# cmeraki/audiotoken

Hardware: AMD Instinct MI355X
Metric: audio-sec tokenized / wall-sec (acoustic + semantic_m) (higher is better)
Workload: dtype f32 (linear layers: two fp16 pieces per operand, three MFMA products, fp32 accumulate)

## Files before the change

audiotoken_amd/_cabi.py:

```python
from __future__ import annotations

import ctypes as C
import os
from pathlib import Path

import numpy as np

_LIB_PATH = Path(__file__).resolve().parent / "lib" / "libaudiotoken_hip.so"
_lib = None


class HipLibraryError(RuntimeError):
    pass


class SegmentDesc(C.Structure):
    _fields_ = [("pcm", C.c_void_p), ("table", C.c_void_p), ("chunk_off", C.c_int64), ("chunk_len", C.c_int32), ("out_start", C.c_int32),
                ("valid_len", C.c_int32), ("fmt", C.c_int32), ("scale", C.c_float), ("o", C.c_int32), ("n", C.c_int32), ("width", C.c_int32),
                ("chunk_out_len", C.c_int32)]


PCM_S16, PCM_S32, PCM_F32, PCM_U8 = 0, 1, 2, 3


class ResampleRow(C.Structure):
    _fields_ = [("pcm", C.c_void_p), ("table", C.c_void_p), ("src_base", C.c_int64), ("src_len", C.c_int64), ("src_total", C.c_int64),
                ("out_start", C.c_int64), ("out_len", C.c_int32), ("fmt", C.c_int32), ("scale", C.c_float), ("o", C.c_int32), ("n", C.c_int32),
                ("width", C.c_int32), ("final", C.c_int32), ("reserved", C.c_int32), ("dst_off", C.c_int64)]


class PcmRowDesc(C.Structure):
    _fields_ = [("src_off", C.c_int64), ("dst_off", C.c_int64), ("n", C.c_int64), ("scale", C.c_float), ("reserved", C.c_int32)]


class FlacRowDesc(C.Structure):
    _fields_ = [("src_off", C.c_int64), ("n", C.c_int64), ("first_block", C.c_int32), ("scale", C.c_float)]


class FlacBlock(C.Structure):
    _fields_ = [("first", C.c_int64), ("byte_off", C.c_int64), ("row", C.c_int32), ("n", C.c_int32), ("kind", C.c_int32), ("order", C.c_int32),
                ("porder", C.c_int32), ("nbytes", C.c_int32)]


FLAC_BLOCK = 4096
FLAC_CONSTANT, FLAC_VERBATIM, FLAC_FIXED = 0, 1, 2
FLAC_BLOCK_DTYPE = np.dtype([("first", "<i8"), ("byte_off", "<i8"), ("row", "<i4"), ("n", "<i4"), ("kind", "<i4"), ("order", "<i4"), ("porder", "<i4"),
                             ("nbytes", "<i4")])


class GemmDesc(C.Structure):
    _fields_ = [
        ("X", C.c_void_p), ("x_bstride", C.c_int64), ("Tin", C.c_int32), ("Cin", C.c_int32), ("ldx", C.c_int32),
        ("ktaps", C.c_int32), ("stride", C.c_int32), ("pad_left", C.c_int32), ("pad_mode", C.c_int32),
        ("W", C.c_void_p), ("bias", C.c_void_p),
        ("C", C.c_void_p), ("c_bstride", C.c_int64), ("ldc", C.c_int32),
        ("R", C.c_void_p), ("r_bstride", C.c_int64), ("ldr", C.c_int32),
        ("M", C.c_int32), ("N", C.c_int32), ("K", C.c_int32), ("batch", C.c_int32),
        ("pro", C.c_int32), ("epi", C.c_int32), ("alpha", C.c_float),
        ("aux_off", C.c_int32), ("row_mask", C.c_void_p),
    ]


SIGNATURES = {
    "at_version": (C.c_int, []),
    "at_last_error": (C.c_char_p, []),
    "at_encodec_create": (C.c_void_p, [C.c_int]),
    "at_encodec_set_tensor": (C.c_int, [C.c_void_p, C.c_char_p, C.c_void_p, C.POINTER(C.c_int64), C.c_int]),
    "at_encodec_finalize": (C.c_int, [C.c_void_p, C.c_int]),
    "at_encodec_destroy": (None, [C.c_void_p]),
    "at_encodec_num_codebooks": (C.c_int, [C.c_void_p]),
    "at_encodec_workspace_bytes": (C.c_size_t, [C.c_void_p, C.c_int, C.c_int]),
    "at_encodec_encode": (C.c_int, [C.c_void_p, C.c_void_p, C.c_void_p, C.c_int, C.c_int, C.c_int, C.c_void_p,
                                    C.POINTER(C.c_int), C.c_void_p, C.c_void_p, C.c_size_t, C.c_void_p]),
    "at_encodec_encode_checked": (C.c_int, [C.c_void_p, C.c_void_p, C.c_void_p, C.c_int, C.c_int, C.c_int, C.c_void_p,
                                            C.POINTER(C.c_int), C.c_void_p, C.c_void_p, C.c_size_t, C.c_void_p, C.c_void_p]),
    "at_encodec_stream_state_bytes": (C.c_size_t, [C.c_void_p, C.c_int]),
    "at_encodec_stream_reset": (C.c_int, [C.c_void_p, C.c_void_p, C.c_int, C.c_void_p]),
    "at_encodec_stream_workspace_bytes": (C.c_size_t, [C.c_void_p, C.c_int, C.c_int]),
    "at_encodec_encode_stream_checked": (C.c_int, [C.c_void_p, C.c_void_p, C.c_void_p, C.c_void_p, C.c_int, C.c_int, C.c_int, C.c_int, C.c_void_p,
                                                   C.POINTER(C.c_int), C.c_void_p, C.c_void_p, C.c_size_t, C.c_void_p, C.c_void_p]),
    "at_encodec_set_option": (C.c_int, [C.c_void_p, C.c_char_p, C.c_int]),
    "at_encodec_profile": (C.c_int, [C.c_void_p, C.c_int]),
    "at_encodec_profile_read": (C.c_int, [C.c_void_p, C.c_char_p, C.c_size_t, C.POINTER(C.c_float), C.POINTER(C.c_int), C.c_int]),
    "at_encodec_decode_workspace_bytes": (C.c_size_t, [C.c_void_p, C.c_int, C.c_int]),
    "at_encodec_decode": (C.c_int, [C.c_void_p, C.c_void_p, C.c_int, C.c_int, C.c_int, C.c_void_p, C.c_void_p,
                                    C.c_size_t, C.c_void_p]),
    "at_encodec_decode_checked": (C.c_int, [C.c_void_p, C.c_void_p, C.c_int, C.c_int, C.c_int, C.c_void_p, C.c_void_p,
                                            C.c_size_t, C.c_void_p, C.c_void_p]),
    "at_encodec_decode_stream_state_bytes": (C.c_size_t, [C.c_void_p, C.c_int]),
    "at_encodec_decode_stream_reset": (C.c_int, [C.c_void_p, C.c_void_p, C.c_int, C.c_void_p]),
    "at_encodec_decode_stream_workspace_bytes": (C.c_size_t, [C.c_void_p, C.c_int, C.c_int]),
    "at_encodec_decode_stream_checked": (C.c_int, [C.c_void_p, C.c_void_p, C.c_void_p, C.c_void_p, C.c_int, C.c_int, C.c_int, C.c_void_p,
                                                   C.c_void_p, C.c_size_t, C.c_void_p, C.c_void_p]),
    "at_encodec_stream_gather": (C.c_int, [C.c_void_p, C.c_void_p, C.c_int, C.c_void_p, C.c_void_p, C.c_int, C.c_void_p, C.c_void_p]),
    "at_encodec_stream_scatter": (C.c_int, [C.c_void_p, C.c_void_p, C.c_int, C.c_void_p, C.c_void_p, C.c_void_p, C.c_int, C.c_void_p]),
    "at_encodec_decode_stream_gather": (C.c_int, [C.c_void_p, C.c_void_p, C.c_int, C.c_void_p, C.c_void_p, C.c_int, C.c_void_p, C.c_void_p]),
    "at_encodec_decode_stream_scatter": (C.c_int, [C.c_void_p, C.c_void_p, C.c_int, C.c_void_p, C.c_void_p, C.c_void_p, C.c_int, C.c_void_p]),
    "at_w2vbert_create": (C.c_void_p, [C.c_int]),
    "at_w2vbert_set_tensor": (C.c_int, [C.c_void_p, C.c_char_p, C.c_void_p, C.POINTER(C.c_int64), C.c_int]),
    "at_w2vbert_finalize": (C.c_int, [C.c_void_p]),
    "at_w2vbert_packed_bytes": (C.c_int64, [C.c_void_p]),
    "at_w2vbert_packed_meta": (C.c_int64, [C.c_void_p, C.c_void_p, C.c_int64]),
    "at_w2vbert_export_packed": (C.c_int, [C.c_void_p, C.c_void_p, C.c_int64, C.c_void_p]),
    "at_w2vbert_import_packed": (C.c_int, [C.c_void_p, C.c_void_p, C.c_int64, C.c_void_p, C.c_int64, C.c_void_p]),
    "at_w2vbert_destroy": (None, [C.c_void_p]),
    "at_w2vbert_num_layers": (C.c_int, [C.c_void_p]),
    "at_w2vbert_num_tokens": (C.c_int, [C.c_int, C.c_int]),
    "at_w2vbert_workspace_bytes": (C.c_size_t, [C.c_void_p, C.c_int, C.c_int, C.c_int]),
    "at_w2vbert_encode": (C.c_int, [C.c_void_p, C.c_void_p, C.c_void_p, C.c_int, C.c_int, C.c_int, C.c_int, C.c_void_p,
                                    C.POINTER(C.c_int), C.c_void_p, C.c_void_p, C.c_void_p, C.c_void_p, C.c_size_t, C.c_void_p]),
    "at_w2vbert_encode_checked": (C.c_int, [C.c_void_p, C.c_void_p, C.c_void_p, C.c_int, C.c_int, C.c_int, C.c_int, C.c_void_p,
                                            C.POINTER(C.c_int), C.c_void_p, C.c_void_p, C.c_void_p, C.c_void_p, C.c_size_t, C.c_void_p, C.c_void_p]),
    "at_w2vbert_set_option": (C.c_int, [C.c_void_p, C.c_char_p, C.c_int]),
    "at_w2vbert_get_option": (C.c_int, [C.c_void_p, C.c_char_p]),
    "at_encodec_get_option": (C.c_int, [C.c_void_p, C.c_char_p]),
    "at_w2vbert_profile": (C.c_int, [C.c_void_p, C.c_int]),
    "at_w2vbert_profile_read": (C.c_int, [C.c_void_p, C.c_char_p, C.c_size_t, C.POINTER(C.c_float), C.POINTER(C.c_int), C.c_int]),
    "at_hubert_create": (C.c_void_p, [C.c_int]),
    "at_hubert_set_tensor": (C.c_int, [C.c_void_p, C.c_char_p, C.c_void_p, C.POINTER(C.c_int64), C.c_int]),
    "at_hubert_finalize": (C.c_int, [C.c_void_p]),
    "at_hubert_packed_bytes": (C.c_int64, [C.c_void_p]),
    "at_hubert_packed_meta": (C.c_int64, [C.c_void_p, C.c_void_p, C.c_int64]),
    "at_hubert_export_packed": (C.c_int, [C.c_void_p, C.c_void_p, C.c_int64, C.c_void_p]),
    "at_hubert_import_packed": (C.c_int, [C.c_void_p, C.c_void_p, C.c_int64, C.c_void_p, C.c_int64, C.c_void_p]),
    "at_hubert_destroy": (None, [C.c_void_p]),
    "at_hubert_num_layers": (C.c_int, [C.c_void_p]),
    "at_hubert_num_tokens": (C.c_int, [C.c_int]),
    "at_hubert_workspace_bytes": (C.c_size_t, [C.c_void_p, C.c_int, C.c_int]),
    "at_hubert_encode": (C.c_int, [C.c_void_p, C.c_void_p, C.c_void_p, C.c_int, C.c_int, C.c_int, C.c_void_p, C.POINTER(C.c_int),
                                   C.c_void_p, C.c_void_p, C.c_size_t, C.c_void_p]),
    "at_hubert_encode_checked": (C.c_int, [C.c_void_p, C.c_void_p, C.c_void_p, C.c_int, C.c_int, C.c_int, C.c_void_p, C.POINTER(C.c_int),
                                           C.c_void_p, C.c_void_p, C.c_size_t, C.c_void_p, C.c_void_p]),
    "at_hubert_features": (C.c_int, [C.c_void_p, C.c_void_p, C.c_int, C.c_int, C.c_void_p, C.c_void_p, C.c_size_t, C.c_void_p, C.c_void_p]),
    "at_op_hub_conv0": (C.c_int, [C.c_void_p, C.c_void_p, C.c_void_p, C.c_void_p, C.c_void_p, C.c_int, C.c_int, C.c_void_p, C.c_size_t, C.c_void_p]),
    "at_op_hub_frame_mask": (C.c_int, [C.c_void_p, C.c_void_p, C.c_int, C.c_int, C.c_int, C.c_void_p]),
    "at_hubert_set_option": (C.c_int, [C.c_void_p, C.c_char_p, C.c_int]),
    "at_hubert_get_option": (C.c_int, [C.c_void_p, C.c_char_p]),
    "at_hubert_profile": (C.c_int, [C.c_void_p, C.c_int]),
    "at_hubert_profile_read": (C.c_int, [C.c_void_p, C.c_char_p, C.c_size_t, C.POINTER(C.c_float), C.POINTER(C.c_int), C.c_int]),
    "at_encodec_range_sites": (C.c_int, [C.c_char_p, C.c_size_t]),
    "at_encodec_range_report": (C.c_int, [C.c_void_p, C.POINTER(C.c_float), C.c_int]),
    "at_w2vbert_range_sites": (C.c_int, [C.c_char_p, C.c_size_t]),
    "at_w2vbert_range_report": (C.c_int, [C.c_void_p, C.POINTER(C.c_float), C.c_int]),
    "at_w2vbert_site_scales": (C.c_int, [C.c_void_p, C.POINTER(C.c_float), C.c_int]),
    "at_hubert_site_scales": (C.c_int, [C.c_void_p, C.POINTER(C.c_float), C.c_int]),
    "at_w2vbert_layer_status": (C.c_int, [C.c_void_p, C.POINTER(C.c_int32), C.c_int]),
    "at_hubert_layer_status": (C.c_int, [C.c_void_p, C.POINTER(C.c_int32), C.c_int]),
    "at_hubert_range_sites": (C.c_int, [C.c_char_p, C.c_size_t]),
    "at_hubert_range_report": (C.c_int, [C.c_void_p, C.POINTER(C.c_float), C.c_int]),
    "at_segments_from_pcm": (C.c_int, [C.c_void_p, C.c_int, C.c_int, C.c_float, C.c_void_p, C.c_void_p, C.c_void_p]),
    "at_clock_stamp": (C.c_int, [C.c_void_p, C.c_void_p]),
    "at_resample_rows": (C.c_int, [C.c_void_p, C.c_int, C.c_void_p, C.c_void_p]),
    "at_resample_rows_check": (C.c_int, [C.c_void_p, C.c_int]),
    "at_segments_zmuv_workspace_bytes": (C.c_size_t, [C.c_int, C.c_int]),
    "at_segments_from_pcm_zmuv": (C.c_int, [C.c_void_p, C.c_int, C.c_int, C.c_int, C.c_float, C.c_float, C.c_void_p, C.c_void_p, C.c_void_p, C.c_size_t, C.c_void_p]),
    "at_pcm_peaks": (C.c_int, [C.c_void_p, C.c_void_p, C.c_int, C.c_int64, C.c_void_p, C.c_void_p]),
    "at_pcm_pack": (C.c_int, [C.c_void_p, C.c_void_p, C.c_int, C.c_int64, C.c_float, C.c_void_p, C.c_void_p, C.c_void_p]),
    "at_flac_encode_workspace_bytes": (C.c_size_t, [C.c_int]),
    "at_flac_encode_rows": (C.c_int, [C.c_void_p, C.c_void_p, C.c_int, C.c_int, C.c_float, C.c_void_p, C.c_void_p, C.c_int64, C.c_void_p, C.c_void_p, C.c_size_t,
                                      C.c_void_p]),
    "at_flac_encode_pcm16": (C.c_int64, [C.c_void_p, C.c_int64, C.c_int, C.c_void_p, C.c_int64, C.c_void_p, C.c_int64, C.c_int64]),
    "at_flac_write_frames": (C.c_int64, [C.c_void_p, C.c_int, C.c_void_p, C.c_int64, C.c_int, C.c_void_p, C.c_int, C.c_void_p, C.c_int64, C.c_void_p]),
    "at_flac_streaminfo": (C.c_int, [C.c_int, C.c_int, C.c_int, C.c_int, C.c_int, C.c_int64, C.c_void_p]),
    "at_flac_info": (C.c_int, [C.c_void_p, C.c_size_t, C.POINTER(C.c_int), C.POINTER(C.c_int), C.POINTER(C.c_int), C.POINTER(C.c_int64), C.c_void_p]),
    "at_flac_decode": (C.c_int64, [C.c_void_p, C.c_size_t, C.c_void_p, C.c_int64]),
    "at_op_layernorm": (C.c_int, [C.c_void_p, C.c_void_p, C.c_void_p, C.c_void_p, C.c_void_p, C.c_int64, C.c_int, C.c_void_p]),
    "at_op_relpos_attention": (C.c_int, [C.c_void_p, C.c_void_p, C.c_void_p, C.c_void_p, C.c_int, C.c_int, C.c_void_p]),
    "at_op_relpos_attention_kvp": (C.c_int, [C.c_void_p, C.c_void_p, C.c_void_p, C.c_float, C.c_void_p, C.c_int, C.c_int, C.c_int, C.c_int, C.c_void_p, C.c_size_t,
                                             C.c_void_p, C.c_void_p]),
    "at_op_dwconv_ln_swish": (C.c_int, [C.c_void_p, C.c_void_p, C.c_void_p, C.c_void_p, C.c_void_p, C.c_int, C.c_int, C.c_void_p]),
    "at_op_dwconv_stream": (C.c_int, [C.c_void_p, C.c_void_p, C.c_void_p, C.c_void_p, C.c_void_p, C.c_int, C.c_int, C.c_void_p]),
    "at_op_vq_argmax": (C.c_int, [C.c_void_p, C.c_void_p, C.c_void_p, C.c_void_p, C.c_int64, C.c_int, C.c_int, C.c_void_p]),
    "at_op_vq_argmax_refined": (C.c_int, [C.c_void_p, C.c_void_p, C.c_void_p, C.c_void_p, C.c_void_p, C.c_int64, C.c_int, C.c_int, C.c_void_p]),
    "at_kmeans_device_bytes": (C.c_size_t, [C.c_int64, C.c_int, C.c_int]),
    "at_kmeans_create": (C.c_void_p, [C.c_int, C.c_int64, C.c_int, C.c_int]),
    "at_kmeans_destroy": (None, [C.c_void_p]),
    "at_kmeans_set_option": (C.c_int, [C.c_void_p, C.c_char_p, C.c_int]),
    "at_kmeans_get_option": (C.c_int, [C.c_void_p, C.c_char_p]),
    "at_kmeans_set_data": (C.c_int, [C.c_void_p, C.c_void_p, C.c_float, C.c_void_p]),
    "at_kmeans_plusplus": (C.c_int, [C.c_void_p, C.c_void_p, C.c_int, C.c_void_p, C.c_void_p, C.c_void_p]),
    "at_kmeans_assign": (C.c_int, [C.c_void_p, C.c_void_p, C.c_float, C.c_void_p, C.c_void_p, C.c_void_p]),
    "at_kmeans_update": (C.c_int, [C.c_void_p, C.c_void_p, C.c_void_p, C.c_void_p, C.c_void_p, C.c_void_p, C.c_void_p, C.c_void_p]),
    "at_kmeans_layernorm": (C.c_int, [C.c_void_p, C.c_void_p, C.c_int64, C.c_int, C.c_int, C.c_void_p, C.c_size_t, C.c_void_p]),
    "at_kmeans_row_d2": (C.c_int, [C.c_void_p, C.c_void_p, C.c_void_p]),
    "at_kmeans_relocations": (C.c_int, [C.c_void_p, C.c_void_p, C.c_void_p]),
    "at_op_gemm": (C.c_int, [C.POINTER(GemmDesc), C.c_void_p]),
    "at_op_gemm_dual": (C.c_int, [C.POINTER(GemmDesc), C.c_void_p, C.c_int64, C.c_int, C.c_int, C.c_void_p]),
    "at_op_gemm_route": (C.c_int, [C.POINTER(GemmDesc), C.c_void_p, C.c_int64, C.c_int, C.c_int, C.POINTER(C.c_int32)]),
    "at_op_attention_f32": (C.c_int, [C.c_void_p, C.c_void_p, C.c_void_p, C.c_void_p, C.c_int, C.c_int, C.c_int, C.c_void_p]),
    "at_required_tensors": (C.c_int, [C.c_char_p, C.c_int, C.c_int, C.c_char_p, C.c_size_t]),
    "at_op_gemm_split": (C.c_int, [C.c_void_p, C.c_void_p, C.c_void_p, C.c_void_p, C.c_int, C.c_int, C.c_int, C.c_int, C.c_float, C.c_int,
                                   C.c_void_p, C.c_size_t, C.c_void_p, C.c_void_p]),
    "at_op_conv_split": (C.c_int, [C.c_void_p, C.c_void_p, C.c_void_p, C.c_void_p, C.c_int, C.c_int, C.c_int, C.c_int, C.c_int, C.c_int, C.c_float,
                                  C.c_void_p, C.c_size_t, C.c_void_p, C.c_void_p]),
    "at_op_rvq_encode_split": (C.c_int, [C.c_void_p, C.c_int64, C.c_int, C.c_void_p, C.c_void_p, C.c_int, C.c_void_p, C.c_int, C.c_float,
                                        C.c_void_p, C.c_size_t, C.c_void_p, C.c_void_p]),
    "at_op_rvq_encode": (C.c_int, [C.c_void_p, C.c_int64, C.c_int, C.c_void_p, C.c_void_p, C.c_int, C.c_void_p, C.c_void_p]),
    "at_gpt_create": (C.c_void_p, [C.c_int]),
    "at_gpt_set_tensor": (C.c_int, [C.c_void_p, C.c_char_p, C.c_void_p, C.POINTER(C.c_int64), C.c_int]),
    "at_gpt_finalize": (C.c_int, [C.c_void_p]),
    "at_gpt_destroy": (None, [C.c_void_p]),
    "at_gpt_num_layers": (C.c_int, [C.c_void_p]),
    "at_gpt_vocab": (C.c_int, [C.c_void_p]),
    "at_gpt_block_size": (C.c_int, [C.c_void_p]),
    "at_gpt_state_bytes": (C.c_size_t, [C.c_void_p, C.c_int, C.c_int]),
    "at_gpt_generate": (C.c_int, [C.c_void_p, C.c_void_p, C.c_int, C.POINTER(C.c_int32), C.c_int, C.c_int, C.c_float, C.c_int, C.c_int, C.c_void_p,
                                  C.POINTER(C.c_int32), C.c_void_p, C.c_void_p, C.c_void_p, C.c_void_p, C.c_void_p, C.c_size_t, C.c_int, C.c_void_p, C.c_void_p]),
    "at_gpt_long_num_windows": (C.c_int, [C.c_int, C.c_int, C.c_int]),
    "at_gpt_long_state_bytes": (C.c_size_t, [C.c_void_p, C.c_int, C.c_int]),
    "at_gpt_generate_long": (C.c_int, [C.c_void_p, C.c_void_p, C.c_int, C.POINTER(C.c_int32), C.c_int, C.c_int, C.c_int, C.c_int, C.c_int, C.c_int, C.c_int,
                                       C.c_int, C.c_int, C.c_int, C.c_int, C.c_float, C.c_int, C.c_void_p, C.c_int, C.c_void_p, C.c_int, C.c_void_p, C.c_void_p,
                                       C.c_void_p, C.c_void_p, C.c_size_t, C.c_int, C.c_void_p, C.c_void_p]),
    "at_gpt_queue_state_bytes": (C.c_size_t, [C.c_void_p, C.c_int, C.c_int, C.c_int]),
    "at_gpt_generate_queue": (C.c_int, [C.c_void_p, C.c_void_p, C.c_int, C.POINTER(C.c_int32), C.c_int, C.c_int, C.c_int, C.c_int, C.c_int, C.c_int, C.c_int,
                                        C.c_int, C.c_int, C.c_int, C.c_int, C.c_float, C.c_int, C.c_void_p, C.c_int, C.c_void_p, C.c_int, C.c_void_p, C.c_void_p,
                                        C.c_void_p, C.c_void_p, C.c_size_t, C.c_int, C.c_int, C.c_int, C.POINTER(C.c_int32), C.c_int, C.POINTER(C.c_int32),
                                        C.POINTER(C.c_int32), C.c_void_p, C.c_void_p]),
    "at_gpt_long_num_windows_prompted": (C.c_int, [C.c_int, C.c_int, C.c_int, C.c_int]),
    "at_gpt_generate_long_prompted": (C.c_int, [C.c_void_p, C.c_void_p, C.c_int, C.POINTER(C.c_int32), C.c_int, C.c_void_p, C.c_int, C.c_void_p, C.c_int,
                                                C.POINTER(C.c_int32), C.c_int, C.POINTER(C.c_int32), C.c_int, C.c_int, C.c_int, C.c_int, C.c_int, C.c_int,
                                                C.c_int, C.c_int, C.c_int, C.c_int, C.c_float, C.c_int, C.c_void_p, C.c_int, C.c_void_p, C.c_int, C.c_void_p,
                                                C.c_void_p, C.c_void_p, C.c_void_p, C.c_size_t, C.c_int, C.c_void_p, C.c_void_p]),
    "at_gpt_generate_queue_prompted": (C.c_int, [C.c_void_p, C.c_void_p, C.c_int, C.POINTER(C.c_int32), C.c_int, C.c_void_p, C.c_int, C.c_void_p, C.c_int,
                                                 C.POINTER(C.c_int32), C.c_int, C.POINTER(C.c_int32), C.c_int, C.c_int, C.c_int, C.c_int, C.c_int, C.c_int,
                                                 C.c_int, C.c_int, C.c_int, C.c_int, C.c_float, C.c_int, C.c_void_p, C.c_int, C.c_void_p, C.c_int, C.c_void_p,
                                                 C.c_void_p, C.c_void_p, C.c_void_p, C.c_size_t, C.c_int, C.c_int, C.c_int, C.POINTER(C.c_int32), C.c_int,
                                                 C.POINTER(C.c_int32), C.POINTER(C.c_int32), C.c_void_p, C.c_void_p]),
    "at_op_topk_sample": (C.c_int, [C.c_void_p, C.c_int, C.c_int, C.c_float, C.c_int, C.c_void_p, C.POINTER(C.c_int32), C.c_void_p, C.c_void_p]),
    "at_gpt_set_truncation": (C.c_int, [C.c_void_p, C.c_float, C.c_float]),
    "at_op_nucleus_sample": (C.c_int, [C.c_void_p, C.c_int, C.c_int, C.c_float, C.c_int, C.c_float, C.c_float, C.c_void_p, C.POINTER(C.c_int32), C.c_void_p,
                                       C.c_void_p, C.c_void_p, C.c_void_p]),
    "at_gpt_score_state_bytes": (C.c_size_t, [C.c_void_p, C.c_int, C.c_int, C.c_int, C.c_int]),
    "at_gpt_score": (C.c_int, [C.c_void_p, C.c_void_p, C.c_int, C.POINTER(C.c_int32), C.POINTER(C.c_int32), C.c_int, C.c_float, C.POINTER(C.c_int32),
                               C.c_void_p, C.c_void_p, C.c_int, C.c_void_p, C.c_void_p, C.c_size_t, C.c_int, C.c_int, C.c_int, C.c_int, C.c_void_p, C.c_void_p]),
    "at_op_score_rows": (C.c_int, [C.c_void_p, C.c_int, C.c_int, C.c_void_p, C.c_float, C.POINTER(C.c_int32), C.c_void_p, C.c_void_p, C.c_void_p]),
    "at_fine_create": (C.c_void_p, [C.c_int]),
    "at_fine_set_tensor": (C.c_int, [C.c_void_p, C.c_char_p, C.c_void_p, C.POINTER(C.c_int64), C.c_int]),
    "at_fine_finalize": (C.c_int, [C.c_void_p]),
    "at_fine_destroy": (None, [C.c_void_p]),
    "at_fine_num_layers": (C.c_int, [C.c_void_p]),
    "at_fine_hidden": (C.c_int, [C.c_void_p]),
    "at_fine_block_size": (C.c_int, [C.c_void_p]),
    "at_fine_has_bias": (C.c_int, [C.c_void_p]),
    "at_fine_num_windows": (C.c_int, [C.c_void_p, C.c_int]),
    "at_fine_state_bytes": (C.c_size_t, [C.c_void_p, C.c_int, C.c_int]),
    "at_fine_generate": (C.c_int, [C.c_void_p, C.c_void_p, C.c_int, C.POINTER(C.c_int32), C.c_int, C.c_float, C.c_int, C.c_void_p, C.c_int, C.c_void_p,
                                   C.c_void_p, C.c_void_p, C.c_void_p, C.c_size_t, C.c_int, C.c_void_p, C.c_void_p]),
    "at_fine_queue_state_bytes": (C.c_size_t, [C.c_void_p, C.c_int, C.c_int]),
    "at_fine_generate_queue": (C.c_int, [C.c_void_p, C.c_void_p, C.POINTER(C.c_int32), C.c_int, C.c_float, C.c_int, C.c_void_p, C.c_void_p, C.c_void_p,
                                         C.c_void_p, C.c_void_p, C.c_size_t, C.c_int, C.c_int, C.POINTER(C.c_int32), C.c_int, C.POINTER(C.c_int32),
                                         C.POINTER(C.c_int32), C.c_void_p, C.c_void_p]),
    "at_fine_num_windows_hist": (C.c_int, [C.c_void_p, C.c_int, C.c_int]),
    "at_fine_state_bytes_hist": (C.c_size_t, [C.c_void_p, C.c_int, C.c_int, C.c_int]),
    "at_fine_queue_state_bytes_hist": (C.c_size_t, [C.c_void_p, C.c_int, C.c_int, C.c_int]),
    "at_fine_generate_hist": (C.c_int, [C.c_void_p, C.c_void_p, C.c_int, C.POINTER(C.c_int32), C.c_int, C.c_void_p, C.c_int, C.POINTER(C.c_int32), C.c_int,
                                        C.POINTER(C.c_int32), C.c_int, C.c_float, C.c_int, C.c_void_p, C.c_int, C.c_void_p, C.c_void_p, C.c_void_p, C.c_void_p,
                                        C.c_size_t, C.c_int, C.c_void_p, C.c_void_p]),
    "at_fine_generate_queue_hist": (C.c_int, [C.c_void_p, C.c_void_p, C.POINTER(C.c_int32), C.c_int, C.c_void_p, C.c_int, C.POINTER(C.c_int32), C.c_int,
                                              C.POINTER(C.c_int32), C.c_int, C.c_float, C.c_int, C.c_void_p, C.c_void_p, C.c_void_p, C.c_void_p, C.c_void_p,
                                              C.c_size_t, C.c_int, C.c_int, C.POINTER(C.c_int32), C.c_int, C.POINTER(C.c_int32), C.POINTER(C.c_int32),
                                              C.c_void_p, C.c_void_p]),
    "at_gpt_stream_state_bytes": (C.c_size_t, [C.c_void_p, C.c_int, C.c_int, C.c_int]),
    "at_gpt_stream_push": (C.c_int, [C.c_void_p, C.c_void_p, C.c_size_t, C.POINTER(C.c_int64), C.c_void_p, C.c_int, C.c_int, C.c_int, C.c_int, C.c_int, C.c_int,
                                     C.c_int, C.c_int, C.c_int, C.c_int, C.c_int, C.c_int, C.c_float, C.c_int, C.c_void_p, C.c_int64, C.c_int64, C.c_void_p,
                                     C.c_int, C.c_void_p, C.c_void_p, C.POINTER(C.c_int32), C.c_void_p, C.c_void_p]),
    "at_fine_stream_state_bytes": (C.c_size_t, [C.c_void_p]),
    "at_fine_stream_push": (C.c_int, [C.c_void_p, C.c_void_p, C.c_size_t, C.POINTER(C.c_int64), C.c_void_p, C.c_int, C.c_int, C.c_int, C.c_int, C.c_float,
                                      C.c_int, C.c_void_p, C.c_int, C.c_int, C.c_void_p, C.c_int, C.POINTER(C.c_int32), C.POINTER(C.c_int32), C.c_void_p,
                                      C.c_void_p]),
    "at_op_fine_handover": (C.c_int, [C.c_void_p, C.c_int, C.c_int, C.c_int, C.c_int, C.c_void_p, C.c_void_p, C.c_void_p]),
    "at_gpt_pool_state_bytes": (C.c_size_t, [C.c_void_p, C.c_int, C.c_int, C.c_int, C.c_int, C.c_int, C.c_int, C.c_int]),
    "at_gpt_pool_push": (C.c_int, [C.c_void_p, C.c_void_p, C.c_size_t, C.c_int, C.c_int, C.c_int, C.c_int, C.POINTER(C.c_int64), C.c_int, C.POINTER(C.c_int32),
                                   C.c_void_p, C.POINTER(C.c_int32), C.POINTER(C.c_int32), C.c_int, C.c_int, C.c_int, C.c_int, C.c_int, C.c_int, C.c_int, C.c_int,
                                   C.c_int, C.c_int, C.c_float, C.c_int, C.c_void_p, C.c_int, C.POINTER(C.c_int64), C.c_void_p, C.c_int, C.c_void_p, C.c_void_p,
                                   C.c_void_p, C.POINTER(C.c_int32), C.POINTER(C.c_int32), C.c_int, C.POINTER(C.c_int32), C.POINTER(C.c_int32),
                                   C.POINTER(C.c_int32), C.c_void_p, C.c_void_p]),
    "at_fine_pool_state_bytes": (C.c_size_t, [C.c_void_p, C.c_int, C.c_int]),
    "at_fine_pool_push": (C.c_int, [C.c_void_p, C.c_void_p, C.c_size_t, C.c_int, C.c_int, C.POINTER(C.c_int64), C.c_int, C.POINTER(C.c_int32), C.c_void_p,
                                    C.POINTER(C.c_int64), C.POINTER(C.c_int32), C.POINTER(C.c_int32), C.c_int, C.c_int, C.c_float, C.c_int, C.c_void_p,
                                    C.POINTER(C.c_int32), C.POINTER(C.c_int32), C.POINTER(C.c_int32), C.c_void_p, C.c_int, C.POINTER(C.c_int32),
                                    C.POINTER(C.c_int32), C.POINTER(C.c_int32), C.c_int, C.POINTER(C.c_int32), C.c_void_p, C.c_void_p]),
}


def lib_path() -> Path:
    return Path(os.environ.get("AUDIOTOKEN_HIP_LIB", str(_LIB_PATH)))


def load():
    global _lib
    if _lib is not None:
        return _lib
    path = lib_path()
    if not path.exists():
        raise HipLibraryError(
            f"{path} not found: build it with `python -c 'import __graft_entry__ as g; g.build()'` "
            f"(or `make -C audiotoken_amd/csrc`). audiotoken_amd has no CPU fallback.")
    try:
        lib = C.CDLL(str(path))
    except OSError as e:
        raise HipLibraryError(f"cannot load {path}: {e}") from e
    for name, (restype, argtypes) in SIGNATURES.items():
        try:
            fn = getattr(lib, name)
        except AttributeError as e:
            raise HipLibraryError(f"{path} does not export {name}") from e
        fn.restype = restype
        fn.argtypes = argtypes
    _lib = lib
    return lib


def required_tensors(model: str, n: int, with_extras: bool = True):
    lib = load()
    need = -lib.at_required_tensors(model.encode(), n, 1 if with_extras else 0, None, 0)
    if need <= 1:
        raise HipLibraryError(f"at_required_tensors({model}) failed: {last_error()}")
    buf = C.create_string_buffer(need)
    cnt = lib.at_required_tensors(model.encode(), n, 1 if with_extras else 0, buf, need)
    out = {}
    for line in buf.value.decode().splitlines():
        parts = line.split()
        out[parts[0]] = tuple(int(x) for x in parts[1:])
    assert len(out) == cnt
    return out


def last_error() -> str:
    msg = load().at_last_error()
    return msg.decode("utf-8", "replace") if msg else ""


def check(rc: int, what: str):
    if rc != 0:
        raise HipLibraryError(f"{what} failed (code {rc}): {last_error()}")


def ptr(t) -> int:
    return 0 if t is None else t.data_ptr()


def current_stream_handle(device) -> int:
    import torch

    return torch.cuda.current_stream(device).cuda_stream


def set_tensor(lib, fn, handle, name: str, arr: np.ndarray):
    arr = np.ascontiguousarray(arr, dtype=np.float32)
    shape = (C.c_int64 * arr.ndim)(*arr.shape)
    check(fn(handle, name.encode(), arr.ctypes.data_as(C.c_void_p), shape, arr.ndim), f"set_tensor({name})")


def range_report(lib, model: str, handle) -> dict:
    names = C.create_string_buffer(2048)
    n = getattr(lib, f"at_{model}_range_sites")(names, 2048)
    if n < 0:
        raise HipLibraryError(f"at_{model}_range_sites failed")
    vals = (C.c_float * 64)()
    check(getattr(lib, f"at_{model}_range_report")(handle, vals, 64) - n, f"at_{model}_range_report")
    keys = names.value.decode().split("\n")[:n]
    return {k: float(vals[i]) for i, k in enumerate(keys)}


def export_packed(lib, model: str, handle, device):
    import torch
    n = getattr(lib, f"at_{model}_packed_meta")(handle, None, 0)
    if n < 0:
        raise HipLibraryError(f"at_{model}_packed_meta failed: {last_error()}")
    buf = C.create_string_buffer(int(n))
    if getattr(lib, f"at_{model}_packed_meta")(handle, buf, n) != n:
        raise HipLibraryError(f"at_{model}_packed_meta failed: {last_error()}")
    nbytes = getattr(lib, f"at_{model}_packed_bytes")(handle)
    if nbytes < 0:
        raise HipLibraryError(f"at_{model}_packed_bytes failed: {last_error()}")
    blob = torch.empty(int(nbytes), dtype=torch.uint8, device=device)
    with torch.cuda.device(device):
        check(getattr(lib, f"at_{model}_export_packed")(handle, blob.data_ptr(), int(nbytes), current_stream_handle(device)), f"at_{model}_export_packed")
        torch.cuda.current_stream(device).synchronize()
    return buf.raw, blob


def import_packed(lib, model: str, handle, meta: bytes, blob) -> None:
    import torch
    assert blob.dtype == torch.uint8 and blob.is_cuda and blob.is_contiguous()
    with torch.cuda.device(blob.device):
        check(getattr(lib, f"at_{model}_import_packed")(handle, meta, len(meta), blob.data_ptr(), blob.numel(), current_stream_handle(blob.device)),
              f"at_{model}_import_packed")
```

audiotoken_amd/csrc/attention_f16x2_w8.hip:

```cpp
#include "at_common.h"
#include "w2vbert_kernels.h"
#include "split_scheme.h"

#include <cstdio>
#include <type_traits>

namespace at {

typedef __attribute__((address_space(3))) void w8_lds_void;

#ifdef W8_DEBUG_STAMPS
__device__ unsigned long long w8_stamps[2][12];
#define W8_T(i) const unsigned long long w8_t##i = __builtin_readcyclecounter()
#define W8_ACC(k, a_, b_) w8_d[k] += w8_t##b_ - w8_t##a_
#else
#define W8_T(i) do {} while (0)
#define W8_ACC(k, a_, b_) do {} while (0)
#endif

constexpr int W8_QB = 256, W8_KB = 64;
constexpr int W8_PLANE_B = W8_KB * 64 * 2;
constexpr int W8_TILE_B = 2 * W8_PLANE_B;
constexpr int W8_KBUFS = 2, W8_VBUFS = 2;
constexpr int W8_KV_B = (W8_KBUFS + W8_VBUFS) * W8_TILE_B;
constexpr int W8_QE_LD = 73;
constexpr int W8_LDS_MAX = 163840;
constexpr float W8_SCALE2 = 0.125f * 1.4426950408889634f;
constexpr float W8_P_LOG2 = 10.0f;
constexpr float W8_DEFER = 4.0f;
#ifndef W8_P_PIECES
#define W8_P_PIECES 2
#endif
constexpr int W8_PP = W8_P_PIECES;

static size_t w8_lds_bytes(int T, bool relpos) {
    const int nkt = (T + W8_KB - 1) / W8_KB;
    return (size_t)W8_KV_B + (relpos ? (size_t)W8_QB * W8_QE_LD * 4 : 0) + (size_t)nkt * W8_KB * 4 + 16;
}

__device__ __forceinline__ float w8_pair_max(float x) {
    const auto r = __builtin_amdgcn_permlane32_swap(__float_as_uint(x), __float_as_uint(x), false, false);
    return fmaxf(__uint_as_float(r[0]), __uint_as_float(r[1]));
}
__device__ __forceinline__ float w8_pair_sum(float x) {
    const auto r = __builtin_amdgcn_permlane32_swap(__float_as_uint(x), __float_as_uint(x), false, false);
    return __uint_as_float(r[0]) + __uint_as_float(r[1]);
}

__device__ __forceinline__ void w8_split_pair(float p0, float p1, unsigned& hi, unsigned& lo) {
    asm("v_cvt_pk_f16_f32 %0, %1, %2" : "=v"(hi) : "v"(p0), "v"(p1));
    asm("v_fma_mixlo_f16 %0, -%1, 1.0, %2 op_sel:[0,0,0] op_sel_hi:[1,0,0]" : "=v"(lo) : "v"(hi), "v"(p0));
    asm("v_fma_mixhi_f16 %0, -%1, 1.0, %2 op_sel:[1,0,0] op_sel_hi:[1,0,0]" : "+v"(lo) : "v"(hi), "v"(p1));
}

constexpr int W8_NQB = 1;
template <bool RELPOS>
__global__ __launch_bounds__(512 / W8_NQB, W8_NQB == 1 ? 2 : 1) void relpos_attention_w8_kernel(const float* __restrict__ qkv, const float* __restrict__ amask,
                                                                     const _Float16* __restrict__ dist_pieces, float dist_inv_scale, float* __restrict__ ctx, int T, int hid,
                                                                     int* __restrict__ status, _Float16* __restrict__ ctx_pieces, long long rows_pad,
                                                                     int nheads, int nclips, const _Float16* __restrict__ kv_pieces) {
    constexpr int NQB = W8_NQB;
    typedef SchemeF16x2 SC;
    typedef _Float16 PT;
    typedef f16x8 V8;
    typedef f16x4 V4;
    constexpr float XS = XB_F16_ACT_SCALE;
    constexpr float S_SCALE2 = W8_SCALE2 / (XS * XS);
    RangeMax over;
    extern __shared__ __attribute__((aligned(16))) unsigned char smem_raw[];
    const int nkt = (T + W8_KB - 1) / W8_KB;
    unsigned char* KV = smem_raw;
    float* QE = reinterpret_cast<float*>(KV + W8_KV_B);
    float* kbt = QE + (RELPOS ? W8_QB * W8_QE_LD : 0);
    int* tmask = reinterpret_cast<int*>(kbt + nkt * W8_KB);
    const int tid = threadIdx.x, lane = tid & 63;
    constexpr int NW = 8 / NQB, QW = 32 * NQB, NT = 64 * NW;
    const int wave = __builtin_amdgcn_readfirstlane(tid >> 6);
    const int l32 = lane & 31, hh = lane >> 5;
    const int nqt = (T + W8_QB - 1) / W8_QB;
    const int nblk = gridDim.x, per_xcd = (nblk + 7) >> 3;
    const int lid = (int)(blockIdx.x & 7) * per_xcd + (int)(blockIdx.x >> 3);
    if (lid >= nqt * nheads * nclips) return;
    const int qt = lid % nqt, pair = lid / nqt;
    const int h = pair % nheads, b = pair / nheads;
    const int l0 = qt * W8_QB;
    const long long rowbase = (long long)b * T;
    const int LD = 3 * hid;
    const float* qp = qkv + h * 64;

    const unsigned plane_b = (unsigned)(rows_pad * (long long)hid * 2);
    const __amdgpu_buffer_rsrc_t kvrs = __builtin_amdgcn_make_buffer_rsrc((void*)kv_pieces, 0, (int)(4u * plane_b), 0x00020000);
    constexpr int RW = 8 * NQB;
    const int d_row = wave * RW + (lane >> 3), d_cs = lane & 7;
    const unsigned clip_b = (unsigned)(rowbase * hid * 2 + h * 128);
    const int row_b = hid * 2;
    auto issue_k = [&](int kt, int buf) {
#pragma unroll
        for (int j = 0; j < NQB; ++j) {
            const int row = min(kt * W8_KB + d_row + 8 * j, T - 1);
            const unsigned vo = clip_b + (unsigned)(row * row_b) + ((d_cs ^ (((d_row + 8 * j) >> 1) & 7)) << 4);
#pragma unroll
            for (int p = 0; p < 2; ++p)
                __builtin_amdgcn_raw_ptr_buffer_load_lds(kvrs, (w8_lds_void*)(KV + buf * W8_TILE_B + wave * (RW * 128) + p * W8_PLANE_B + j * 1024), 16, vo, p * plane_b, 0, 0);
        }
    };
    auto issue_v = [&](int kt, int buf) {
#pragma unroll
        for (int j = 0; j < NQB; ++j) {
            const int row = min(kt * W8_KB + d_row + 8 * j, T - 1);
            const unsigned vo = clip_b + (unsigned)(row * row_b) + ((d_cs ^ ((((d_row + 8 * j) >> 1) & 1) << 2)) << 4);
#pragma unroll
            for (int p = 0; p < 2; ++p)
                __builtin_amdgcn_raw_ptr_buffer_load_lds(kvrs, (w8_lds_void*)(KV + (W8_KBUFS + buf) * W8_TILE_B + wave * (RW * 128) + p * W8_PLANE_B + j * 1024), 16, vo,
                                                         (2u + p) * plane_b, 0, 0);
        }
    };
    issue_k(0, 0);
    issue_v(0, 0);
    if (nkt > 1) issue_k(1, 1);

    const float FMIN = -3.4028234663852886e38f;
    if (tid < 2) tmask[tid] = 0;
    __syncthreads();
    for (int k = tid; k < nkt * W8_KB; k += NT) {
        float v = -INFINITY;
        if (k < T) v = amask[rowbase + k] != 0.f ? 0.f : FMIN;
        kbt[k] = v;
        if (v != 0.f) atomicOr(&tmask[k >> 11], 1 << ((k >> 6) & 31));
    }
    const int lq0 = l0 + wave * QW + l32;
    V8 qpc[NQB][2][4];
#pragma unroll
    for (int qb = 0; qb < NQB; ++qb) {
        const int lq = lq0 + 32 * qb;
        const int lc = lq < T ? lq : T - 1;
#pragma unroll
        for (int ds = 0; ds < 4; ++ds) {
            const f4 a = *reinterpret_cast<const f4*>(qp + (rowbase + lc) * LD + ds * 16 + 8 * hh);
            const f4 c = *reinterpret_cast<const f4*>(qp + (rowbase + lc) * LD + ds * 16 + 8 * hh + 4);
            V4 pa[2], pc[2];
            over |= split4<SC>(a, XS, pa);
            over |= split4<SC>(c, XS, pc);
#pragma unroll
            for (int i = 0; i < 2; ++i)
#pragma unroll
                for (int k = 0; k < 4; ++k) { qpc[qb][i][ds][k] = pa[i][k]; qpc[qb][i][ds][4 + k] = pc[i][k]; }
        }
    }
    if constexpr (RELPOS) {
        const float qe_scale = W8_SCALE2 * dist_inv_scale / XS;
#pragma unroll
        for (int qb = 0; qb < NQB; ++qb) {
            float* row = QE + (wave * QW + qb * 32 + l32) * W8_QE_LD;
#pragma unroll
            for (int rt = 0; rt < 3; ++rt) {
                f16v acc;
#pragma unroll
                for (int r = 0; r < 16; ++r) acc[r] = 0.f;
#pragma unroll
                for (int ds = 0; ds < 4; ++ds) {
                    V8 ef[2];
#pragma unroll
                    for (int p = 0; p < 2; ++p) ef[p] = *reinterpret_cast<const V8*>(dist_pieces + (p * 96 + rt * 32 + l32) * 64 + ds * 16 + 8 * hh);
#pragma unroll
                    for (int t = 0; t < SC::NPROD; ++t) acc = SC::mfma(ef[SC::prod_a(t)], qpc[qb][SC::prod_w(t)][ds], acc);
                }
#pragma unroll
                for (int r = 0; r < 16; ++r) {
                    const int bucket = rt * 32 + 8 * (r >> 2) + 4 * hh + (r & 3);
                    if (bucket < W8_QE_LD) row[bucket] = qe_scale * acc[r];
                }
            }
        }
    }
    f16v oacc[NQB][2];
#pragma unroll
    for (int qb = 0; qb < NQB; ++qb)
#pragma unroll
        for (int dt = 0; dt < 2; ++dt)
#pragma unroll
            for (int r = 0; r < 16; ++r) oacc[qb][dt][r] = 0.f;
    float mrun[NQB], lrun[NQB], alpha[NQB];
    bool rescale[NQB];
#pragma unroll
    for (int qb = 0; qb < NQB; ++qb) { mrun[qb] = -INFINITY; lrun[qb] = 0.f; alpha[qb] = 0.f; }
    const int wl_min = l0 + wave * QW, wl_max = wl_min + QW - 1;
    int koff[4];
#pragma unroll
    for (int ds = 0; ds < 4; ++ds) koff[ds] = l32 * 128 + (((2 * ds + hh) ^ ((l32 >> 1) & 7)) << 4);
    int voff[2];
    {
        const int li = lane & 15, vq = li >> 2, vp = li & 3;
        const int c0 = ((lane & 16) >> 3) + (vp >> 1), sv = (vq >> 1) & 1;
#pragma unroll
        for (int dt = 0; dt < 2; ++dt) voff[dt] = (4 * hh + vq) * 128 + ((((dt ^ sv) << 2) + c0) << 4) + (vp & 1) * 8;
    }
    asm volatile("s_waitcnt vmcnt(0)" ::: "memory");
    __syncthreads();
    const int tm0 = __builtin_amdgcn_readfirstlane(tmask[0]), tm1 = __builtin_amdgcn_readfirstlane(tmask[1]);
    typedef const __attribute__((address_space(3))) float lds_cf;
    typedef const __attribute__((address_space(3))) f4 lds_cf4;
    lds_cf* qe0 = (lds_cf*)(QE + (wave * QW + l32) * W8_QE_LD);
    lds_cf* kbt3 = (lds_cf*)kbt;
    float c_left[NQB], c_right[NQB];
#pragma unroll
    for (int qb = 0; qb < NQB; ++qb) { c_left[qb] = 0.f; c_right[qb] = 0.f; }
    if constexpr (RELPOS) {
#pragma unroll
        for (int qb = 0; qb < NQB; ++qb) { c_left[qb] = qe0[qb * 32 * W8_QE_LD]; c_right[qb] = qe0[qb * 32 * W8_QE_LD + 72]; }
    }

    auto s_tile = [&](f16v (&s)[NQB][2], int kbuf) {
        const unsigned char* Kb = KV + kbuf * W8_TILE_B;
#pragma unroll
        for (int kh = 0; kh < 2; ++kh) {
#pragma unroll
            for (int qb = 0; qb < NQB; ++qb)
#pragma unroll
                for (int r = 0; r < 16; ++r) s[qb][kh][r] = 0.f;
#pragma unroll
            for (int ds = 0; ds < 4; ++ds) {
                V8 kf[2];
#pragma unroll
                for (int p = 0; p < 2; ++p) kf[p] = *reinterpret_cast<const V8*>(Kb + p * W8_PLANE_B + kh * 32 * 128 + koff[ds]);
#pragma unroll
                for (int t = 0; t < SC::NPROD; ++t)
#pragma unroll
                    for (int qb = 0; qb < NQB; ++qb) s[qb][kh] = SC::mfma(kf[SC::prod_a(t)], qpc[qb][SC::prod_w(t)][ds], s[qb][kh]);
            }
        }
    };
    auto tile_fast = [&](int kt, bool& far_left) -> bool {
        const int r0 = kt * W8_KB;
        far_left = (r0 + W8_KB - 1) - wl_min <= -64;
        const bool far_right = r0 - wl_max >= 8;
        const bool masked = (((kt < 32 ? tm0 : tm1) >> (kt & 31)) & 1) != 0;
        return (!RELPOS || far_left || far_right) && !masked;
    };
    auto bias_pass = [&](f16v (&s)[2], int r0, int lq, lds_cf* qe, float c_far, auto near_) -> float {
        constexpr bool NEAR = decltype(near_)::value;
        float mx = -INFINITY;
#pragma unroll
        for (int kh = 0; kh < 2; ++kh)
#pragma unroll
            for (int g = 0; g < 4; ++g) {
                const int key0 = kh * 32 + 8 * g + 4 * hh;
                const f4 kb4 = *(lds_cf4*)(kbt3 + r0 + key0);
#pragma unroll
                for (int e = 0; e < 4; ++e) {
                    float bias = c_far;
                    if constexpr (NEAR) {
                        int dd = (r0 + key0 + e) - lq;
                        dd = dd < -64 ? -64 : (dd > 8 ? 8 : dd);
                        bias = qe[dd + 64];
                    }
                    const float sc = fmaf(S_SCALE2, s[kh][4 * g + e], bias + kb4[e]);
                    s[kh][4 * g + e] = sc;
                    mx = fmaxf(mx, sc);
                }
            }
        return mx;
    };
    auto softmax_general = [&](f16v (&s)[2], int kt, int qb) {
        const int r0 = kt * W8_KB;
        const int bmin = wl_min + 32 * qb, bmax = bmin + 31;
        const bool far_left = (r0 + W8_KB - 1) - bmin <= -64;
        const bool far_right = r0 - bmax >= 8;
        float mx;
        if (!RELPOS || far_left || far_right) mx = bias_pass(s, r0, 0, qe0, far_left ? c_left[qb] : c_right[qb], std::false_type{});
        else mx = bias_pass(s, r0, lq0 + 32 * qb, qe0 + qb * 32 * W8_QE_LD, 0.f, std::true_type{});
        mx = w8_pair_max(mx);
        const bool resc = __builtin_amdgcn_ballot_w64(mx > mrun[qb] + W8_DEFER) != 0ull;
        rescale[qb] = resc;
        const float mnew = resc ? fmaxf(mrun[qb], mx) : mrun[qb];
        const float sub = mnew - W8_P_LOG2;
        float rs = 0.f;
#pragma unroll
        for (int kh = 0; kh < 2; ++kh)
#pragma unroll
            for (int r = 0; r < 16; ++r) {
                const float p = __builtin_amdgcn_exp2f(s[kh][r] - sub);
                s[kh][r] = p;
                rs += p;
            }
        rs = w8_pair_sum(rs);
        alpha[qb] = resc ? __builtin_amdgcn_exp2f(mrun[qb] - mnew) : 1.0f;
        lrun[qb] = lrun[qb] * alpha[qb] + rs;
        mrun[qb] = mnew;
    };
    float f_mraw[NQB], f_mnew[NQB], f_bias2[NQB], f_rs[NQB], f_cfar[NQB];
    auto stat_slice = [&](f16v (&sa)[2], int qb, int k) {
        if (k < 4) {
            if (k == 0) { f_mraw[qb] = -INFINITY; f_rs[qb] = 0.f; }
#pragma unroll
            for (int e = 0; e < 8; ++e) f_mraw[qb] = fmaxf(f_mraw[qb], sa[k >> 1][8 * (k & 1) + e]);
        } else if (k == 4) {
            const float mx = w8_pair_max(fmaf(S_SCALE2, f_mraw[qb], f_cfar[qb]));
            const bool resc = __builtin_amdgcn_ballot_w64(mx > mrun[qb] + W8_DEFER) != 0ull;
            rescale[qb] = resc;
            f_mnew[qb] = resc ? fmaxf(mrun[qb], mx) : mrun[qb];
            f_bias2[qb] = (f_cfar[qb] - f_mnew[qb]) + W8_P_LOG2;
            alpha[qb] = resc ? __builtin_amdgcn_exp2f(mrun[qb] - f_mnew[qb]) : 1.0f;
        } else if (k < 21) {
#pragma unroll
            for (int e = 0; e < 2; ++e) {
                const int r = 2 * (k - 5) + e;
                const float p = __builtin_amdgcn_exp2f(fmaf(S_SCALE2, sa[r >> 4][r & 15], f_bias2[qb]));
                sa[r >> 4][r & 15] = p;
                f_rs[qb] += p;
            }
        } else if (k == 21) {
            const float rs = w8_pair_sum(f_rs[qb]);
            lrun[qb] = lrun[qb] * alpha[qb] + rs;
            mrun[qb] = f_mnew[qb];
        }
    };
    auto s_tile_softmax = [&](f16v (&sb)[NQB][2], int kbuf, f16v (&sa)[NQB][2]) {
        const unsigned char* Kb = KV + kbuf * W8_TILE_B;
        V8 kf[3][2];
        auto load_k = [&](int g) {
#pragma unroll
            for (int p = 0; p < 2; ++p) kf[g % 3][p] = *reinterpret_cast<const V8*>(Kb + p * W8_PLANE_B + (g >> 2) * 32 * 128 + koff[g & 3]);
        };
        load_k(0);
        load_k(1);
#pragma unroll
        for (int qb = 0; qb < NQB; ++qb)
#pragma unroll
            for (int kh = 0; kh < 2; ++kh)
#pragma unroll
                for (int r = 0; r < 16; ++r) sb[qb][kh][r] = 0.f;
        __builtin_amdgcn_sched_barrier(0);
#pragma unroll
        for (int g = 0; g < 8; ++g) {
            if (g + 2 < 8) load_k(g + 2);
#pragma unroll
            for (int t = 0; t < SC::NPROD; ++t)
#pragma unroll
                for (int qb = 0; qb < NQB; ++qb) {
                    sb[qb][g >> 2] = SC::mfma(kf[g % 3][SC::prod_a(t)], qpc[qb][SC::prod_w(t)][g & 3], sb[qb][g >> 2]);
                    const int sl = (3 * g + t) * NQB + qb;
                    if (sl < 22) stat_slice(sa[0], 0, sl);
                    else if (NQB > 1 && sl < 44) stat_slice(sa[NQB - 1], NQB - 1, sl - 22);
                    __builtin_amdgcn_sched_barrier(0);
                }
        }
    };
    auto pv_split = [&](const f16v (&s)[NQB][2], int vbuf) {
        const unsigned char* Vb = KV + (W8_KBUFS + vbuf) * W8_TILE_B;
        typedef short s4_ __attribute__((__vector_size__(4 * sizeof(short))));
        typedef unsigned u4_ __attribute__((ext_vector_type(4)));
        u4_ pp[2][NQB][2];
        auto split_pair = [&](int ks, int qb, int j) {
            unsigned hi, lo;
            if constexpr (W8_PP == 2) {
                w8_split_pair(s[qb][ks >> 1][8 * (ks & 1) + j], s[qb][ks >> 1][8 * (ks & 1) + j + 1], hi, lo);
                pp[ks & 1][qb][1][j >> 1] = lo;
            } else {
                asm("v_cvt_pk_f16_f32 %0, %1, %2" : "=v"(hi) : "v"(s[qb][ks >> 1][8 * (ks & 1) + j]), "v"(s[qb][ks >> 1][8 * (ks & 1) + j + 1]));
            }
            pp[ks & 1][qb][0][j >> 1] = hi;
        };
        V8 vf[2][2];
        auto load_v = [&](int u) {
#pragma unroll
            for (int p = 0; p < 2; ++p) {
                const unsigned char* vb = Vb + p * W8_PLANE_B + (u >> 1) * 16 * 128 + voff[u & 1];
                const s4_ lo = __builtin_amdgcn_ds_read_tr16_b64_v4i16((__attribute__((address_space(3))) s4_*)(vb));
                const s4_ hi = __builtin_amdgcn_ds_read_tr16_b64_v4i16((__attribute__((address_space(3))) s4_*)(vb + 8 * 128));
#pragma unroll
                for (int k = 0; k < 4; ++k) {
                    vf[u & 1][p][k] = __builtin_bit_cast(PT, (short)lo[k]);
                    vf[u & 1][p][4 + k] = __builtin_bit_cast(PT, (short)hi[k]);
                }
            }
        };
        load_v(0);
#pragma unroll
        for (int qb = 0; qb < NQB; ++qb)
#pragma unroll
            for (int j = 0; j < 8; j += 2) split_pair(0, qb, j);
        asm volatile("s_nop 1");
        __builtin_amdgcn_sched_barrier(0);
#pragma unroll
        for (int u = 0; u < 8; ++u) {
            const int ks = u >> 1, dt = u & 1;
            if (u + 1 < 8) load_v(u + 1);
            constexpr int T0 = W8_PP == 2 ? 0 : 1;
#pragma unroll
            for (int t = T0; t < SC::NPROD; ++t)
#pragma unroll
                for (int qb = 0; qb < NQB; ++qb) {
                    oacc[qb][dt] = SC::mfma(vf[u & 1][SC::prod_a(t)], __builtin_bit_cast(V8, pp[ks & 1][qb][SC::prod_w(t)]), oacc[qb][dt]);
                    const int sl = (dt * (SC::NPROD - T0) + (t - T0)) * NQB + qb;
                    if (ks + 1 < 4 && sl < 4 * NQB) split_pair(ks + 1, sl >> 2, 2 * (sl & 3));
                    __builtin_amdgcn_sched_barrier(0);
                }
        }
    };
#ifdef W8_DEBUG_STAMPS
    unsigned long long w8_d[8] = {0, 0, 0, 0, 0, 0, 0, 0};
    const unsigned long long w8_begin = __builtin_readcyclecounter();
#endif
    auto interval = [&](int i, f16v (&sa)[NQB][2], f16v (&sb)[NQB][2]) {
        W8_T(0);
        asm volatile("s_waitcnt vmcnt(0)" ::: "memory");
        W8_T(1);
        __builtin_amdgcn_s_barrier();
        W8_T(2);
        const bool more = i + 1 < nkt;
        if (i + 2 < nkt) issue_k(i + 2, i & 1);
        if (more) issue_v(i + 1, (i + 1) & 1);
        bool far_left;
        const bool fast = tile_fast(i, far_left);
        W8_T(3);
        if (more && fast) {
#pragma unroll
            for (int qb = 0; qb < NQB; ++qb) f_cfar[qb] = far_left ? c_left[qb] : c_right[qb];
            s_tile_softmax(sb, (i + 1) & 1, sa);
        } else {
            if (more) s_tile(sb, (i + 1) & 1);
            __builtin_amdgcn_sched_barrier(0);
            if (fast) {
#pragma unroll
                for (int qb = 0; qb < NQB; ++qb) {
                    f_cfar[qb] = far_left ? c_left[qb] : c_right[qb];
#pragma unroll
                    for (int k = 0; k < 22; ++k) stat_slice(sa[qb], qb, k);
                }
            } else {
#pragma unroll
                for (int qb = 0; qb < NQB; ++qb) softmax_general(sa[qb], i, qb);
            }
        }
        __builtin_amdgcn_sched_barrier(0);
        W8_T(4);
#pragma unroll
        for (int qb = 0; qb < NQB; ++qb)
            if (rescale[qb]) {
#pragma unroll
                for (int dt = 0; dt < 2; ++dt)
#pragma unroll
                    for (int r = 0; r < 16; ++r) oacc[qb][dt][r] *= alpha[qb];
            }
        __builtin_amdgcn_sched_barrier(0);
        W8_T(5);
        pv_split(sa, i & 1);
        W8_T(6);
#ifdef W8_DEBUG_STAMPS
        W8_ACC(0, 0, 1); W8_ACC(1, 1, 2); W8_ACC(2, 2, 3); W8_ACC(fast && more ? 3 : 4, 3, 4); W8_ACC(5, 4, 5); W8_ACC(6, 5, 6);
        w8_d[7] += (fast && more) ? 1 : 0;
#endif
    };
    f16v sA[NQB][2], sB[NQB][2];
    s_tile(sA, 0);
    for (int i = 0; i < nkt; i += 2) {
        interval(i, sA, sB);
        if (i + 1 < nkt) interval(i + 1, sB, sA);
    }
#ifdef W8_DEBUG_STAMPS
    if (blockIdx.x == (gridDim.x / 2) + 8 && (threadIdx.x == 0 || threadIdx.x == NT / 2)) {
        const int g = threadIdx.x ? 1 : 0;
        for (int k = 0; k < 8; ++k) w8_stamps[g][k] = w8_d[k];
        w8_stamps[g][8] = __builtin_readcyclecounter() - w8_begin;
        w8_stamps[g][9] = (unsigned long long)nkt;
    }
#endif
#pragma unroll
    for (int qb = 0; qb < NQB; ++qb) {
        const int lq = lq0 + 32 * qb;
        if (lq < T) {
            const float inv = (1.0f / lrun[qb]) * (1.0f / XS);
#pragma unroll
            for (int dt = 0; dt < 2; ++dt)
#pragma unroll
                for (int g = 0; g < 4; ++g) {
                    const f4 v = {oacc[qb][dt][4 * g] * inv, oacc[qb][dt][4 * g + 1] * inv, oacc[qb][dt][4 * g + 2] * inv, oacc[qb][dt][4 * g + 3] * inv};
                    if (ctx_pieces)
                        over |= store_pieces4<SC>(ctx_pieces, rows_pad * hid, rows_pad, rowbase + lq, h * 64 + dt * 32 + 8 * g + 4 * hh, v, XS);
                    else
                        *reinterpret_cast<f4*>(ctx + (rowbase + lq) * hid + h * 64 + dt * 32 + 8 * g + 4 * hh) = v;
                }
        }
    }
    range_publish(status, status ? status + 1 : nullptr, over);
}

bool relpos_attention_w8_eligible(int T, int heads, long long rows_pad, long long B, bool relpos) {
    return T >= 1 && T <= 4096  && rows_pad * heads * 64 * 8 < (1ll << 32)  && w8_lds_bytes(T, relpos) <= (size_t)W8_LDS_MAX && rows_pad >= B * T && (long long)T * heads * 64 * 2 < (1ll << 31);
}

int launch_relpos_attention_w8(const AttnArgs& a, hipStream_t stream) {
    const float *qkv = a.qkv, *amask = a.amask;
    float* const ctx = a.ctx;
    const int B = a.B, T = a.T, heads = a.heads;
    int* const status = a.status;
    __bf16* const ctx_pieces = a.ctx_pieces;
    const long long rows_pad = a.rows_pad;
    const __bf16 *kv_pieces = a.kv_pieces, *dist_pieces = a.dist.p;
    const float dist_scale = a.dist.s;
    AT_REQUIRE(kv_pieces != nullptr && relpos_attention_w8_eligible(T, heads, rows_pad, B, dist_pieces != nullptr),
               "relpos_attention_w8: needs pre-split k / v and a clip whose key-bias table fits LDS (T <= 1728 with rel-pos)");
    const long long nblk = (long long)((T + W8_QB - 1) / W8_QB) * heads * B;
    dim3 grid((unsigned)((nblk + 7) / 8 * 8));
    const size_t lds = w8_lds_bytes(T, dist_pieces != nullptr);
    const size_t lds_max = W8_LDS_MAX;
    int rc;
    const int hid = heads * 64;
    _Float16* cp = reinterpret_cast<_Float16*>(ctx_pieces);
    const _Float16* kp = reinterpret_cast<const _Float16*>(kv_pieces);
    const _Float16* dp = reinterpret_cast<const _Float16*>(dist_pieces);
    const float dinv = dist_pieces ? 1.0f / dist_scale : 1.0f;
    if (dist_pieces) {
        static LdsAttrFlags lds_attr;
        rc = set_max_dynamic_lds(lds_attr, relpos_attention_w8_kernel<true>, lds_max);
        if (!rc) hipLaunchKernelGGL((relpos_attention_w8_kernel<true>), grid, dim3(512 / W8_NQB), lds, stream, qkv, amask, dp, dinv, ctx, T, hid, status, cp, rows_pad, heads, B, kp);
    } else {
        static LdsAttrFlags lds_attr;
        rc = set_max_dynamic_lds(lds_attr, relpos_attention_w8_kernel<false>, lds_max);
        if (!rc) hipLaunchKernelGGL((relpos_attention_w8_kernel<false>), grid, dim3(512 / W8_NQB), lds, stream, qkv, amask, dp, dinv, ctx, T, hid, status, cp, rows_pad, heads, B, kp);
    }
    if (rc) return rc;
    AT_CHECK_HIP(hipGetLastError());
#ifdef W8_DEBUG_STAMPS
    {
        static int printed = 0;
        if (printed < 3) {
            ++printed;
            (void)hipStreamSynchronize(stream);
            unsigned long long hb[2][12];
            (void)hipMemcpyFromSymbol(hb, HIP_SYMBOL(w8_stamps), sizeof(hb));
            for (int g = 0; g < 2; ++g) {
                const double n = (double)(hb[g][9] ? hb[g][9] : 1), nf = (double)(hb[g][7] ? hb[g][7] : 1), ng = n - hb[g][7] > 0 ? n - hb[g][7] : 1;
                std::fprintf(stderr, "w8 stamps B %d T %d heads %d wave %d (cycles per 64-key interval, 64 queries): dma wait %.0f  barrier %.0f  issue+classify %.0f  phase A fast %.0f (x%llu)  phase A general/last %.0f (x%.0f)  rescale %.0f  phase B %.0f | loop total %.0f per interval, %llu intervals\n",
                             B, T, heads, g * 4, hb[g][0] / n, hb[g][1] / n, hb[g][2] / n, hb[g][3] / nf, hb[g][7], hb[g][4] / ng, ng, hb[g][5] / n, hb[g][6] / n, hb[g][8] / n, hb[g][9]);
            }
        }
    }
#endif
    return 0;
}

__global__ __launch_bounds__(256) void dist_split_kernel(const float* __restrict__ e, _Float16* __restrict__ out, float scale) {
    const int q = blockIdx.x * 256 + threadIdx.x;
    if (q >= 96 * 16) return;
    const int row = q >> 4, col = (q & 15) * 4;
    f4 v = {0.f, 0.f, 0.f, 0.f};
    if (row < 73) v = *reinterpret_cast<const f4*>(e + row * 64 + col);
    SchemeNoCheck<SchemeF16x2>::V4 p[2];
    split4<SchemeNoCheck<SchemeF16x2>>(v, scale, p);
#pragma unroll
    for (int i = 0; i < 2; ++i) *reinterpret_cast<f16x4*>(out + (i * 96 + row) * 64 + col) = p[i];
}
int launch_dist_split(const float* dist_emb, __bf16* out, float scale, hipStream_t stream) {
    hipLaunchKernelGGL(dist_split_kernel, dim3(6), dim3(256), 0, stream, dist_emb, reinterpret_cast<_Float16*>(out), scale);
    AT_CHECK_HIP(hipGetLastError());
    return 0;
}

__global__ __launch_bounds__(256) void kv_rowmajor_split_kernel(const float* __restrict__ qkv, _Float16* __restrict__ out, long long rows, long long rows_pad,
                                                                int hid, int* __restrict__ status) {
    typedef SchemeF16x2 SC;
    const long long q = (long long)blockIdx.x * 256 + threadIdx.x;
    const int qpr = hid / 4;
    RangeMax over;
    if (q < rows * 2 * qpr) {
        const long long row = q / (2 * qpr);
        const int rem = (int)(q - row * 2 * qpr), which = rem / qpr, col = (rem - which * qpr) * 4;
        const f4 v = *reinterpret_cast<const f4*>(qkv + row * 3 * hid + (1 + which) * hid + col);
        SC::V4 p[2];
        over |= split4<SC>(v, XB_F16_ACT_SCALE, p);
#pragma unroll
        for (int i = 0; i < 2; ++i) *reinterpret_cast<SC::V4*>(out + ((long long)(which * 2 + i) * rows_pad + row) * hid + col) = p[i];
    }
    range_publish(status, status ? status + 1 : nullptr, over);
}

int launch_kv_rowmajor_split(const float* qkv, __bf16* out, long long rows, long long rows_pad, int hid, int* status, hipStream_t stream) {
    AT_REQUIRE(hid % 4 == 0 && rows_pad >= rows, "kv_rowmajor_split: bad shape");
    const long long quads = rows * 2 * (hid / 4);
    hipLaunchKernelGGL(kv_rowmajor_split_kernel, dim3((unsigned)((quads + 255) / 256)), dim3(256), 0, stream, qkv, reinterpret_cast<_Float16*>(out), rows, rows_pad, hid,
                       status);
    AT_CHECK_HIP(hipGetLastError());
    return 0;
}

}
```

audiotoken_amd/csrc/semantic_ops.hip:

```cpp
#include "../../include/audiotoken_hip.h"
#include "gemm_bf16x3.h"
#include "w2vbert_kernels.h"

using namespace at;

extern "C" {

int at_op_layernorm(const float* x, const float* gamma, const float* beta, const float* row_mask, float* y, int64_t rows, int D,
                    at_stream_t stream) {
    AT_REQUIRE(x && y, "null pointer");
    return launch_layernorm(x, gamma, beta, row_mask, y, rows, D, (hipStream_t)stream);
}

int at_op_relpos_attention(const float* qkv, const float* attn_mask, const float* dist_emb80, float* ctx, int B, int T,
                           at_stream_t stream) {
    AT_REQUIRE(qkv && attn_mask && dist_emb80 && ctx && B >= 1 && T >= 1, "bad arguments");
    AttnArgs a;
    a.qkv = qkv; a.amask = attn_mask; a.dist_emb = dist_emb80; a.ctx = ctx; a.B = B; a.T = T;
    return launch_relpos_attention(a, (hipStream_t)stream);
}

int at_op_attention_f32(const float* qkv, const float* attn_mask, const float* dist_emb80, float* ctx, int B, int T, int heads, at_stream_t stream) {
    AT_REQUIRE(qkv && attn_mask && ctx && B >= 1 && T >= 1 && heads >= 1 && heads <= 64, "bad arguments");
    AttnArgs a;
    a.qkv = qkv; a.amask = attn_mask; a.dist_emb = dist_emb80; a.ctx = ctx; a.B = B; a.T = T; a.heads = heads; a.arith = 0;
    return launch_relpos_attention(a, (hipStream_t)stream);
}

int at_op_relpos_attention_kvp(const float* qkv, const float* attn_mask, const float* dist_emb80, float dist_max_abs, float* ctx, int B, int T, int heads, int w8,
                               void* kv_workspace, size_t kv_workspace_bytes, int32_t* status_dev, at_stream_t stream) {
    AT_REQUIRE(qkv && attn_mask && ctx && kv_workspace && B >= 1 && T >= 1 && heads >= 1 && heads <= 64, "bad arguments");
    const long long rows = (long long)B * T, rows_pad = (rows + 255) / 256 * 256;
    const int hid = heads * 64;
    const size_t kv_bytes = (size_t)4 * rows_pad * hid * 2, dist_bytes = (size_t)2 * 96 * 64 * 2;
    AT_REQUIRE(kv_workspace_bytes >= kv_bytes + dist_bytes, "kv workspace too small: 4 * ceil256(B * T) * heads * 64 * 2 + 24576 bytes");
    if (int rc = launch_kv_rowmajor_split(qkv, static_cast<__bf16*>(kv_workspace), rows, rows_pad, hid, status_dev, (hipStream_t)stream)) return rc;
    AttnArgs a;
    a.qkv = qkv; a.amask = attn_mask; a.dist_emb = dist_emb80; a.ctx = ctx; a.B = B; a.T = T; a.heads = heads; a.arith = 2;
    a.status = status_dev; a.rows_pad = rows_pad; a.kv_pieces = static_cast<const __bf16*>(kv_workspace); a.w8 = w8;
    if (dist_emb80) {
        __bf16* dist_s = reinterpret_cast<__bf16*>(static_cast<char*>(kv_workspace) + kv_bytes);
        a.dist = SplitW{dist_s, xb_weight_scale(dist_max_abs)};
        if (int rc = launch_dist_split(dist_emb80, dist_s, a.dist.s, (hipStream_t)stream)) return rc;
    }
    return launch_relpos_attention(a, (hipStream_t)stream);
}

int at_op_dwconv_ln_swish(const float* g, const float* w31x1024, const float* gamma, const float* beta, float* out, int B, int T,
                          at_stream_t stream) {
    AT_REQUIRE(g && w31x1024 && gamma && beta && out && B >= 1 && T >= 1, "bad arguments");
    return launch_dwconv_ln_swish(g, w31x1024, gamma, beta, out, B, T, (hipStream_t)stream);
}

int at_op_dwconv_stream(const float* g, const float* w31x1024, const float* gamma, const float* beta, float* out, int B, int T,
                        at_stream_t stream) {
    AT_REQUIRE(g && w31x1024 && gamma && beta && out && B >= 1 && T >= 1, "bad arguments");
    return launch_dwconv_stream(g, w31x1024, gamma, beta, out, B, T, (hipStream_t)stream);
}

int at_op_vq_argmax(const float* x, const float* dots, const float* e2, int16_t* out, int64_t rows, int D, int C, at_stream_t stream) {
    AT_REQUIRE(x && dots && e2 && out && D % 4 == 0 && C % 4 == 0, "bad arguments");
    return launch_vq_argmax(x, dots, e2, out, rows, D, C, (hipStream_t)stream);
}

int at_op_vq_argmax_refined(const float* x, const float* dots, const float* e2, const float* codebook, int16_t* out, int64_t rows, int D, int C, at_stream_t stream) {
    AT_REQUIRE(x && dots && e2 && codebook && out && D % 4 == 0 && C % 4 == 0, "bad arguments");
    return launch_vq_argmax(x, dots, e2, out, rows, D, C, (hipStream_t)stream, nullptr, 0, codebook);
}

}
```

audiotoken_amd/csrc/w2vbert.hip:

```cpp
#include <string>
#include <vector>
#include <cstring>
#include <cmath>

#include "../../include/audiotoken_hip.h"
#include "semantic_handle.h"
#include "w2vbert_kernels.h"

namespace at {
const char* last_error_cstr();
}
using namespace at;

namespace {
constexpr int kHid = 1024, kFfn = 4096, kFeat = 160, kMel = 80, kFrame = 400, kHop = 160;
constexpr int kSpecLd = 520, kImOff = 260, kCodes = 2048, kBuckets = 73;

enum { W_1A = 0, W_1B, W_2A, W_2B, W_QKV, W_O, W_PW1, W_PW2, W_NLINEAR };
constexpr int kWN[W_NLINEAR] = {kFfn, kHid, kFfn, kHid, 3 * kHid, kHid, 2 * kHid, kHid}, kWK[W_NLINEAR] = {kHid, kFfn, kHid, kFfn, kHid, kHid, kHid, kHid};

enum WSite { WS_LN_FFN1 = 0, WS_FFN1_HIDDEN, WS_LN_ATTN, WS_QKV_KV, WS_ATTENTION, WS_LN_CONV, WS_DWCONV, WS_LN_FFN2, WS_FFN2_HIDDEN, WS_OTHER, W_NSITES };
static const char* const kWSiteNames[W_NSITES] = {"ln_ffn1", "ffn1_hidden", "ln_attn", "qkv_kv", "attention", "ln_conv", "dwconv_out", "ln_ffn2", "ffn2_hidden", "other"};
static_assert((int)W_NSITES == 10, "LayerW::site_scale has one entry per WSite");
constexpr int kRangeLayers = 64, kRangeLayer0 = 0;

struct LayerW {
    const float *ln_ffn1_g, *ln_ffn1_b, *w1a, *b1a, *w1b, *b1b;
    const float *ln_att_g, *ln_att_b, *wqkv, *bqkv, *dist, *wo, *bo;
    const float *ln_conv_g, *ln_conv_b, *pw1, *dw, *ln_dw_g, *ln_dw_b, *pw2;
    const float *ln_ffn2_g, *ln_ffn2_b, *w2a, *b2a, *w2b, *b2b;
    const float *ln_fin_g, *ln_fin_b;
    SplitW ws[2][W_NLINEAR];
    SplitW dist_s;
    float site_scale[W_NSITES] = {XB_F16_ACT_SCALE, XB_F16_ACT_SCALE, XB_F16_ACT_SCALE, XB_F16_ACT_SCALE, XB_F16_ACT_SCALE,
                                  XB_F16_ACT_SCALE, XB_F16_ACT_SCALE, XB_F16_ACT_SCALE, XB_F16_ACT_SCALE, XB_F16_ACT_SCALE};
};

struct W2vBertW {
    const float *window = nullptr, *melw = nullptr;
    double* dft64 = nullptr;
    const float *fp_ln_g = nullptr, *fp_ln_b = nullptr, *fp_w = nullptr, *fp_b = nullptr;
    std::vector<LayerW> layers;
    const float *codebook = nullptr, *e2 = nullptr;
    SplitW cb_s[2];
};
}

struct at_w2vbert : SemanticHandle, W2vBertW {
    bool vq_split = true;
    bool dwconv_stream = true;
    explicit at_w2vbert(int device_id) : SemanticHandle(PACKED_MODEL_W2VBERT, device_id, RangeTable{kRangeLayers, (int)W_NSITES, kRangeLayer0}) {
        bool_opts = {{"dwconv_stream", &dwconv_stream}, {"vq_split", &vq_split}};
    }
    int finalize_model() override;
    int split_model(int scheme) override;
    void forget_model() override { static_cast<W2vBertW&>(*this) = W2vBertW{}; }
    int num_layers() const override { return (int)layers.size(); }
    bool has_codes() const override { return codebook != nullptr; }
};

namespace {

int frames_of(int N) { return N >= kFrame ? 1 + (N - kFrame) / kHop : 0; }
int tokens_of(int N, int mult) {
    int t = frames_of(N) / 2;
    if (mult > 0 && t % mult) t += mult - t % mult;
    return t;
}

struct Plan {
    int F, Tp;
    size_t off_frames, off_fmask, off_spec, off_logmel, off_stats, off_feats, off_amask, off_x, off_t1, off_big, off_tok, off_t1s, off_bigs, off_kvs;
    size_t Mpad;
    size_t total_floats;
};

Plan make_plan(int B, int N, int mult) {
    Plan p;
    p.F = frames_of(N);
    p.Tp = tokens_of(N, mult);
    size_t cur = 0;
    auto takef = [&](size_t n) { size_t o = cur; cur += (n + 63) / 64 * 64; return o; };
    const size_t M = (size_t)B * p.Tp, BF = (size_t)B * p.F;
    p.off_frames = takef(BF * kFrame * 2);
    p.off_fmask = takef(BF);
    p.off_spec = takef(BF * kSpecLd);
    p.off_logmel = takef(BF * kMel);
    p.off_stats = takef((size_t)B * 2 * kMel);
    p.off_feats = takef(M * kFeat);
    p.off_amask = takef(M);
    p.off_x = takef(M * kHid);
    p.off_t1 = takef(M * kHid);
    p.off_big = takef(M * kFfn);
    p.off_tok = takef(M);
    p.Mpad = (M + 255) / 256 * 256;
    p.off_t1s = takef(p.Mpad * kHid * 3 / 2);
    p.off_bigs = takef(p.Mpad * kFfn * 3 / 2);
    p.off_kvs = takef(p.Mpad * kHid * 2 * 2 / 2);
    p.total_floats = cur;
    return p;
}

int take_frontend(at_w2vbert* h) {
    const bool imp = h->arena.importing;
    bool ok = true;
    h->window = take(h, "frontend.window", {kFrame}, ok);
    if (!ok) return -1;
    if (int rc = take_repacked(h, (size_t)kMel * kImOff, &h->melw, [&](std::vector<float>& m) {
            const HostTensor* mf = find(h, "frontend.mel_filters");
            AT_REQUIRE(mf && mf->shape == (std::vector<int64_t>{257, kMel}), "frontend.mel_filters [257,80] missing");
            for (int k = 0; k < 257; ++k)
                for (int j = 0; j < kMel; ++j) m[(size_t)j * kImOff + k] = mf->data[(size_t)k * kMel + j];
            return 0;
        }))
        return rc;
    h->dft64 = static_cast<double*>(h->arena.alloc((size_t)kSpecLd * kFrame * sizeof(double)));
    if (imp) {
        AT_REQUIRE(h->melw && h->dft64, "import_packed: front-end tables");
        return 0;
    }
    AT_REQUIRE(h->melw != nullptr && h->dft64 != nullptr, "device allocation failed (front-end tables)");
    std::vector<double> d((size_t)kSpecLd * kFrame, 0.0);
    const double two_pi = 6.283185307179586476925286766559;
    for (int k = 0; k < 257; ++k)
        for (int t = 0; t < kFrame; ++t) {
            const int ph = (int)(((long long)k * t) % 512);
            const double ang = two_pi * ph / 512.0;
            d[(size_t)k * kFrame + t] = std::cos(ang);
            d[(size_t)(kImOff + k) * kFrame + t] = -std::sin(ang);
        }
    AT_CHECK_HIP(hipMemcpy(h->dft64, d.data(), d.size() * sizeof(double), hipMemcpyHostToDevice));
    return 0;
}

int take_attention(at_w2vbert* h, const std::string& p, LayerW& L) {
    static const char* const kQkv[3] = {"linear_q", "linear_k", "linear_v"};
    if (int rc = take_qkv(h, p + ".self_attn.", kQkv, kHid, &L.wqkv, &L.bqkv)) return rc;
    if (int rc = take_repacked(h, (size_t)80 * 64, &L.dist, [&](std::vector<float>& e) {
            const HostTensor* de = find(h, p + ".self_attn.distance_embedding.weight");
            AT_REQUIRE(de && de->shape == (std::vector<int64_t>{kBuckets, 64}), "distance_embedding [73,64] missing");
            std::memcpy(e.data(), de->data.data(), (size_t)kBuckets * 64 * sizeof(float));
            return 0;
        }))
        return rc;
    AT_REQUIRE(L.wqkv && L.bqkv && L.dist, h->arena.importing ? "import_packed: attention tensors" : "device allocation failed");
    return 0;
}

int take_conv_module(at_w2vbert* h, const std::string& p, LayerW& L) {
    if (int rc = take_repacked(h, (size_t)2 * kHid * kHid, &L.pw1, [&](std::vector<float>& w) {
            const HostTensor* pw = find(h, p + ".conv_module.pointwise_conv1.weight");
            AT_REQUIRE(pw && pw->shape == (std::vector<int64_t>{2 * kHid, kHid, 1}), "pointwise_conv1 [2048,1024,1] missing");
            for (int c = 0; c < kHid; ++c) {
                std::memcpy(&w[(size_t)(2 * c) * kHid], &pw->data[(size_t)c * kHid], kHid * sizeof(float));
                std::memcpy(&w[(size_t)(2 * c + 1) * kHid], &pw->data[(size_t)(kHid + c) * kHid], kHid * sizeof(float));
            }
            return 0;
        }))
        return rc;
    if (int rc = take_repacked(h, (size_t)31 * kHid, &L.dw, [&](std::vector<float>& d) {
            const HostTensor* dw = find(h, p + ".conv_module.depthwise_conv.weight");
            AT_REQUIRE(dw && dw->shape == (std::vector<int64_t>{kHid, 1, 31}), "depthwise_conv [1024,1,31] missing");
            for (int c = 0; c < kHid; ++c)
                for (int j = 0; j < 31; ++j) d[(size_t)j * kHid + c] = dw->data[(size_t)c * 31 + j];
            return 0;
        }))
        return rc;
    AT_REQUIRE(L.pw1 && L.dw, h->arena.importing ? "import_packed: conv-module tensors" : "device allocation failed");
    return 0;
}

int take_layer(at_w2vbert* h, int i, LayerW& L) {
    const std::string p = "encoder.layers." + std::to_string(i);
    bool ok = true;
    L.ln_ffn1_g = take(h, p + ".ffn1_layer_norm.weight", {kHid}, ok);
    L.ln_ffn1_b = take(h, p + ".ffn1_layer_norm.bias", {kHid}, ok);
    L.w1a = take(h, p + ".ffn1.intermediate_dense.weight", {kFfn, kHid}, ok);
    L.b1a = take(h, p + ".ffn1.intermediate_dense.bias", {kFfn}, ok);
    L.w1b = take(h, p + ".ffn1.output_dense.weight", {kHid, kFfn}, ok);
    L.b1b = take(h, p + ".ffn1.output_dense.bias", {kHid}, ok);
    L.ln_att_g = take(h, p + ".self_attn_layer_norm.weight", {kHid}, ok);
    L.ln_att_b = take(h, p + ".self_attn_layer_norm.bias", {kHid}, ok);
    if (!ok) return -1;
    if (int rc = take_attention(h, p, L)) return rc;
    L.wo = take(h, p + ".self_attn.linear_out.weight", {kHid, kHid}, ok);
    L.bo = take(h, p + ".self_attn.linear_out.bias", {kHid}, ok);
    L.ln_conv_g = take(h, p + ".conv_module.layer_norm.weight", {kHid}, ok);
    L.ln_conv_b = take(h, p + ".conv_module.layer_norm.bias", {kHid}, ok);
    if (!ok) return -1;
    if (int rc = take_conv_module(h, p, L)) return rc;
    L.ln_dw_g = take(h, p + ".conv_module.depthwise_layer_norm.weight", {kHid}, ok);
    L.ln_dw_b = take(h, p + ".conv_module.depthwise_layer_norm.bias", {kHid}, ok);
    L.pw2 = take(h, p + ".conv_module.pointwise_conv2.weight", {kHid, kHid, 1}, ok);
    L.ln_ffn2_g = take(h, p + ".ffn2_layer_norm.weight", {kHid}, ok);
    L.ln_ffn2_b = take(h, p + ".ffn2_layer_norm.bias", {kHid}, ok);
    L.w2a = take(h, p + ".ffn2.intermediate_dense.weight", {kFfn, kHid}, ok);
    L.b2a = take(h, p + ".ffn2.intermediate_dense.bias", {kFfn}, ok);
    L.w2b = take(h, p + ".ffn2.output_dense.weight", {kHid, kFfn}, ok);
    L.b2b = take(h, p + ".ffn2.output_dense.bias", {kHid}, ok);
    L.ln_fin_g = take(h, p + ".final_layer_norm.weight", {kHid}, ok);
    L.ln_fin_b = take(h, p + ".final_layer_norm.bias", {kHid}, ok);
    if (!ok) return -1;
    L.site_scale[WS_LN_FFN1] = ln_site_scale(h, L.ln_ffn1_g, L.ln_ffn1_b, kHid);
    L.site_scale[WS_LN_ATTN] = ln_site_scale(h, L.ln_att_g, L.ln_att_b, kHid);
    L.site_scale[WS_LN_CONV] = ln_site_scale(h, L.ln_conv_g, L.ln_conv_b, kHid);
    L.site_scale[WS_DWCONV] = ln_site_scale(h, L.ln_dw_g, L.ln_dw_b, kHid);
    L.site_scale[WS_LN_FFN2] = ln_site_scale(h, L.ln_ffn2_g, L.ln_ffn2_b, kHid);
    for (auto it = h->staged.begin(); it != h->staged.end();)
        it = it->first.compare(0, p.size() + 1, p + ".") == 0 ? h->staged.erase(it) : std::next(it);
    return 0;
}

int take_codebook(at_w2vbert* h) {
    if (h->arena.importing) {
        if (h->imp.flags & 1) {
            h->codebook = reserve(h, (size_t)kCodes * kHid);
            h->e2 = reserve(h, kCodes);
            AT_REQUIRE(h->codebook && h->e2, "import_packed: code book");
        }
        return 0;
    }
    const HostTensor* cb = find(h, "vq._codebook.embed");
    if (!cb) return 0;
    AT_REQUIRE((cb->shape == std::vector<int64_t>{1, kCodes, kHid}) || (cb->shape == std::vector<int64_t>{kCodes, kHid}),
               "vq._codebook.embed must be [1,2048,1024]");
    h->codebook = upload(h, cb->data);
    const HostTensor* e = find(h, "vq._codebook.e2");
    if (e) AT_REQUIRE(e->data.size() == (size_t)kCodes, "bad e2 shape");
    h->e2 = upload(h, e ? e->data : code_norms(cb->data, kCodes, kHid));
    AT_REQUIRE(h->codebook && h->e2, "device allocation failed (codebook)");
    return 0;
}

}

int at_w2vbert::split_model(int scheme) {
    for (LayerW& L : layers) {
        const float* src[W_NLINEAR] = {L.w1a, L.w1b, L.w2a, L.w2b, L.wqkv, L.wo, L.pw1, L.pw2};
        for (int j = 0; j < W_NLINEAR; ++j)
            if (int rc = split_one(this, scheme, src[j], kWN[j], kWK[j], &L.ws[scheme][j])) return rc;
        if (scheme == XB_SCHEME_F16X2) {
            piece_t* d = static_cast<piece_t*>(arena.alloc((size_t)2 * 96 * 64 * sizeof(piece_t)));
            if (!d) return -1;
            float s = 1.f;
            if (int rc = weight_scale(this, L.dist, &s)) return rc;
            if (!arena.importing)
                if (int rc = launch_dist_split(L.dist, d, s, nullptr)) return rc;
            L.dist_s = SplitW{d, s};
        }
    }
    if (codebook)
        if (int rc = split_one(this, scheme, codebook, kCodes, kHid, &cb_s[scheme])) return rc;
    return 0;
}

int at_w2vbert::finalize_model() {
    if (int rc = take_frontend(this)) return rc;
    bool ok = true;
    fp_ln_g = take(this, "feature_projection.layer_norm.weight", {kFeat}, ok);
    fp_ln_b = take(this, "feature_projection.layer_norm.bias", {kFeat}, ok);
    fp_w = take(this, "feature_projection.projection.weight", {kHid, kFeat}, ok);
    fp_b = take(this, "feature_projection.projection.bias", {kHid}, ok);
    if (!ok) return -1;
    int nl = arena.importing ? imp.n_layers : 0;
    while (!arena.importing && find(this, "encoder.layers." + std::to_string(nl) + ".ffn1_layer_norm.weight")) ++nl;
    for (int i = 0; i < nl; ++i) {
        LayerW L{};
        if (int rc = take_layer(this, i, L)) return rc;
        layers.push_back(L);
    }
    return take_codebook(this);
}

extern "C" {

at_w2vbert_t* at_w2vbert_create(int device_id) { return device_exists("at_w2vbert_create", device_id) ? new at_w2vbert(device_id) : nullptr; }
int at_w2vbert_set_tensor(at_w2vbert_t* h, const char* name, const float* host_data, const int64_t* shape, int ndim) {
    return stage_tensor(h, name, host_data, shape, ndim);
}
int at_w2vbert_finalize(at_w2vbert_t* h) { return sem_finalize(h); }
int64_t at_w2vbert_packed_bytes(at_w2vbert_t* h) { return sem_packed_bytes(h, "at_w2vbert_packed_bytes"); }
int64_t at_w2vbert_packed_meta(at_w2vbert_t* h, void* host_dst, int64_t cap) { return sem_packed_meta(h, "at_w2vbert_packed_meta", host_dst, cap); }
int at_w2vbert_export_packed(at_w2vbert_t* h, void* device_dst, int64_t bytes, void* stream) {
    return sem_export_packed(h, "at_w2vbert_export_packed", device_dst, bytes, stream);
}
int at_w2vbert_import_packed(at_w2vbert_t* h, const void* host_meta, int64_t meta_bytes, const void* device_src, int64_t bytes, void* stream) {
    return sem_import_packed(h, "at_w2vbert_import_packed", host_meta, meta_bytes, device_src, bytes, stream);
}
void at_w2vbert_destroy(at_w2vbert_t* h) { sem_destroy(h); }

int at_w2vbert_num_layers(const at_w2vbert_t* h) { return h ? (int)h->layers.size() : 0; }
int at_w2vbert_num_tokens(int N, int pad_to_multiple_of) { return tokens_of(N, pad_to_multiple_of); }

size_t at_w2vbert_workspace_bytes(const at_w2vbert_t* h, int B, int N, int pad_to_multiple_of) {
    if (B <= 0 || N < kFrame) return 0;
    return make_plan(B, N, pad_to_multiple_of).total_floats * sizeof(float);
}

int at_w2vbert_profile(at_w2vbert_t* h, int enable) { return profile_enable(h, enable); }
int at_w2vbert_profile_read(at_w2vbert_t* h, char* names, size_t names_cap, float* total_ms, int* launches, int max_groups) {
    return profile_read(h, names, names_cap, total_ms, launches, max_groups);
}

int at_w2vbert_set_option(at_w2vbert_t* h, const char* name, int value) { return sem_set_option(h, "at_w2vbert_set_option", name, value); }
int at_w2vbert_get_option(const at_w2vbert_t* h, const char* name) { return sem_get_option(h, name); }

}

namespace {

struct Call {
    at_w2vbert* h;
    hipStream_t stream;
    int B, N, F, T, n_layers;
    long long M, BF, Mpad;
    int* status;
    double* frames;
    float *fmask, *spec, *logmel, *stats, *feats, *amask, *x, *t1, *big;
    piece_t *t1s, *bigs, *kvs;
    SplitCtx ctx_of(int li) const { return SplitCtx{scheme_of(h->arith_of(li)), h->range.layer_row(li)}; }
};

int linear(const Call& c, const float* X, int K, const float* W, const float* bias, float* C, int N, int epi, float alpha, const float* R, const float* row_mask,
           int ldc) {
    GemmArgs a;
    a.X = X; a.x_bstride = 0; a.Tin = (int)c.M; a.Cin = K; a.ldx = K;
    a.W = W; a.bias = bias; a.C = C; a.ldc = ldc; a.R = R; a.ldr = ldc;
    a.M = (int)c.M; a.N = N; a.K = K; a.batch = 1; a.epi = epi; a.alpha = alpha; a.row_mask = row_mask;
    return launch_gemm(a, c.stream);
}

int a_site_of(int w) {
    switch (w) {
        case W_1A: return WS_LN_FFN1;  case W_1B: return WS_FFN1_HIDDEN;  case W_2A: return WS_LN_FFN2;  case W_2B: return WS_FFN2_HIDDEN;
        case W_QKV: return WS_LN_ATTN; case W_O: return WS_ATTENTION;     case W_PW1: return WS_LN_CONV; default: return WS_DWCONV;
    }
}
int out_site_of(int w) { return w == W_1A ? WS_FFN1_HIDDEN : w == W_2A ? WS_FFN2_HIDDEN : WS_OTHER; }

int gemm_split(const Call& c, const SplitCtx& sc, const LayerW& L, int w, const piece_t* A, const float* bias, int epi, float alpha, float* C, const float* R,
               piece_t* S) {
    const int out_site = out_site_of(w), ldc = epi == XB_EPI_GLU ? kWN[w] / 2 : kWN[w];
    Bf16x3Args a = split_gemm_args(sc.scheme, A, sc.act(L.site_scale[a_site_of(w)]), L.ws[sc.scheme][w], c.M, kWN[w], kWK[w], c.Mpad, epi, sc.site(out_site),
                                   sc.act(L.site_scale[out_site]));
    a.bias = bias; a.C = C; a.ldc = ldc; a.R = R; a.ldr = ldc; a.alpha = alpha; a.S = S; a.Spad = (int)c.Mpad;
    return launch_gemm_bf16x3(a, c.stream);
}

int ln_split(const Call& c, const SplitCtx& sc, const LayerW& L, int site, const float* g, const float* b, const float* row_mask) {
    c.h->prof.begin("layernorm", 1, c.stream);
    if (int rc = launch_layernorm_split(c.x, g, b, row_mask, nullptr, c.M, kHid, sc.out(c.t1s, c.Mpad, L.site_scale[site], sc.site(site)), c.stream)) return rc;
    c.h->prof.end(c.stream);
    return 0;
}

int front_end(const Call& c, const float* wav, const float* mask) {
    const at_w2vbert* h = c.h;
    c.h->prof.begin("frontend", 5, c.stream);
    if (int rc = launch_frame_prep(wav, mask, h->window, c.frames, c.fmask, c.B, c.N, c.F, c.stream, c.status)) return rc;
    if (int rc = launch_dft_f64(c.frames, h->dft64, c.spec, c.BF, kSpecLd, c.stream)) return rc;
    {
        GemmArgs a;
        a.X = c.spec; a.Tin = (int)c.BF; a.Cin = kImOff; a.ldx = kSpecLd; a.W = h->melw; a.C = c.logmel; a.ldc = kMel;
        a.M = (int)c.BF; a.N = kMel; a.K = kImOff; a.batch = 1; a.pro = PRO_POWER; a.aux_off = kImOff; a.epi = EPI_LOGFLOOR;
        if (int rc = launch_gemm(a, c.stream)) return rc;
    }
    if (int rc = launch_fbank_normalize(c.logmel, c.fmask, c.stats, c.feats, c.amask, c.B, c.F, c.T, c.stream)) return rc;
    c.h->prof.end(c.stream);
    return 0;
}

int feature_projection(const Call& c) {
    const at_w2vbert* h = c.h;
    c.h->prof.begin("feature_projection", 2, c.stream);
    if (int rc = launch_layernorm(c.feats, h->fp_ln_g, h->fp_ln_b, nullptr, c.t1, c.M, kFeat, c.stream)) return rc;
    if (int rc = linear(c, c.t1, kFeat, h->fp_w, h->fp_b, c.x, kHid, EPI_NONE, 1.f, nullptr, c.amask, kHid)) return rc;
    c.h->prof.end(c.stream);
    return 0;
}

int attention_split(const Call& c, const SplitCtx& sc, const LayerW& L) {
    Profiler& prof = c.h->prof;
    if (int rc = ln_split(c, sc, L, WS_LN_ATTN, L.ln_att_g, L.ln_att_b, nullptr)) return rc;
    prof.begin("attn_proj", 1, c.stream);
    const bool kvp = sc.scheme == XB_SCHEME_F16X2;
    if (kvp) {
        if (int rc = qkv_split_gemm(sc, WS_QKV_KV, c.t1s, L.site_scale[WS_LN_ATTN], L.ws[sc.scheme][W_QKV], L.bqkv, kHid, c.M, c.Mpad, c.big, c.kvs, c.stream)) return rc;
    } else if (int rc = gemm_split(c, sc, L, W_QKV, c.t1s, L.bqkv, XB_EPI_LINEAR, 1.f, c.big, nullptr, nullptr)) {
        return rc;
    }
    prof.end(c.stream);
    prof.begin("attention", 1, c.stream);
    AttnArgs at;
    at.qkv = c.big; at.amask = c.amask; at.dist_emb = L.dist; at.B = c.B; at.T = c.T; at.heads = 16;
    at.arith = kvp ? ARITH_F16X2 : ARITH_BF16X3;
    at.status = sc.site(WS_ATTENTION); at.ctx_pieces = c.t1s; at.rows_pad = c.Mpad; at.kv_pieces = kvp ? c.kvs : nullptr; at.w8 = c.h->attn_w8; at.dist = L.dist_s;
    if (int rc = launch_relpos_attention(at, c.stream)) return rc;
    prof.end(c.stream);
    prof.begin("attn_proj", 1, c.stream);
    if (int rc = gemm_split(c, sc, L, W_O, c.t1s, L.bo, XB_EPI_LINEAR, 1.f, c.x, c.x, nullptr)) return rc;
    prof.end(c.stream);
    return 0;
}

int conformer_layer_split(const Call& c, int li) {
    at_w2vbert* const h = c.h;
    Profiler& prof = h->prof;
    const LayerW& L = h->layers[li];
    const SplitCtx sc = c.ctx_of(li);
    if (li == 0)
        if (int rc = ln_split(c, sc, L, WS_LN_FFN1, L.ln_ffn1_g, L.ln_ffn1_b, nullptr)) return rc;
    prof.begin("ffn", 2, c.stream);
    if (int rc = gemm_split(c, sc, L, W_1A, c.t1s, L.b1a, XB_EPI_SWISH_SPLIT, 1.f, nullptr, nullptr, c.bigs)) return rc;
    if (int rc = gemm_split(c, sc, L, W_1B, c.bigs, L.b1b, XB_EPI_LINEAR, 0.5f, c.x, c.x, nullptr)) return rc;
    prof.end(c.stream);

    if (int rc = attention_split(c, sc, L)) return rc;

    if (int rc = ln_split(c, sc, L, WS_LN_CONV, L.ln_conv_g, L.ln_conv_b, c.amask)) return rc;
    prof.begin("conv_module", 3, c.stream);
    if (int rc = gemm_split(c, sc, L, W_PW1, c.t1s, nullptr, XB_EPI_GLU, 1.f, c.big, nullptr, nullptr)) return rc;
    if (int rc = (h->dwconv_stream ? launch_dwconv_stream : launch_dwconv_ln_swish)(c.big, L.dw, L.ln_dw_g, L.ln_dw_b, nullptr, c.B, c.T, c.stream,
                                                                                    sc.out(c.t1s, c.Mpad, L.site_scale[WS_DWCONV], sc.site(WS_DWCONV))))
        return rc;
    if (int rc = gemm_split(c, sc, L, W_PW2, c.t1s, nullptr, XB_EPI_LINEAR, 1.f, c.x, c.x, nullptr)) return rc;
    prof.end(c.stream);

    if (int rc = ln_split(c, sc, L, WS_LN_FFN2, L.ln_ffn2_g, L.ln_ffn2_b, nullptr)) return rc;
    prof.begin("ffn", 2, c.stream);
    if (int rc = gemm_split(c, sc, L, W_2A, c.t1s, L.b2a, XB_EPI_SWISH_SPLIT, 1.f, nullptr, nullptr, c.bigs)) return rc;
    if (int rc = gemm_split(c, sc, L, W_2B, c.bigs, L.b2b, XB_EPI_LINEAR, 0.5f, c.x, c.x, nullptr)) return rc;
    prof.end(c.stream);
    prof.begin("layernorm", 1, c.stream);
    if (li + 1 < c.n_layers) {
        const LayerW& Ln = h->layers[li + 1];
        const SplitCtx scn = c.ctx_of(li + 1);
        if (int rc = launch_layernorm2_split(c.x, L.ln_fin_g, L.ln_fin_b, c.x, Ln.ln_ffn1_g, Ln.ln_ffn1_b, c.M, kHid,
                                             scn.out(c.t1s, c.Mpad, Ln.site_scale[WS_LN_FFN1], scn.site(WS_LN_FFN1)), c.stream))
            return rc;
    } else if (int rc = launch_layernorm(c.x, L.ln_fin_g, L.ln_fin_b, nullptr, c.x, c.M, kHid, c.stream)) {
        return rc;
    }
    prof.end(c.stream);
    return 0;
}

int conformer_layer_f32(const Call& c, int li) {
    at_w2vbert* const h = c.h;
    Profiler& prof = h->prof;
    const LayerW& L = h->layers[li];
    prof.begin("ffn", 3, c.stream);
    if (int rc = launch_layernorm(c.x, L.ln_ffn1_g, L.ln_ffn1_b, nullptr, c.t1, c.M, kHid, c.stream)) return rc;
    if (int rc = linear(c, c.t1, kHid, L.w1a, L.b1a, c.big, kFfn, EPI_SWISH, 1.f, nullptr, nullptr, kFfn)) return rc;
    if (int rc = linear(c, c.big, kFfn, L.w1b, L.b1b, c.x, kHid, EPI_NONE, 0.5f, c.x, nullptr, kHid)) return rc;
    prof.end(c.stream);
    prof.begin("attn_proj", 3, c.stream);
    if (int rc = launch_layernorm(c.x, L.ln_att_g, L.ln_att_b, nullptr, c.t1, c.M, kHid, c.stream)) return rc;
    if (int rc = linear(c, c.t1, kHid, L.wqkv, L.bqkv, c.big, 3 * kHid, EPI_NONE, 1.f, nullptr, nullptr, 3 * kHid)) return rc;
    prof.end(c.stream);
    prof.begin("attention", 1, c.stream);
    AttnArgs at;
    at.qkv = c.big; at.amask = c.amask; at.dist_emb = L.dist; at.ctx = c.t1; at.B = c.B; at.T = c.T; at.heads = 16; at.arith = ARITH_F32;
    if (int rc = launch_relpos_attention(at, c.stream)) return rc;
    prof.end(c.stream);
    prof.begin("attn_proj", 0, c.stream);
    if (int rc = linear(c, c.t1, kHid, L.wo, L.bo, c.x, kHid, EPI_NONE, 1.f, c.x, nullptr, kHid)) return rc;
    prof.end(c.stream);
    prof.begin("conv_module", 4, c.stream);
    if (int rc = launch_layernorm(c.x, L.ln_conv_g, L.ln_conv_b, c.amask, c.t1, c.M, kHid, c.stream)) return rc;
    if (int rc = linear(c, c.t1, kHid, L.pw1, nullptr, c.big, 2 * kHid, EPI_GLU, 1.f, nullptr, nullptr, kHid)) return rc;
    if (int rc = (h->dwconv_stream ? launch_dwconv_stream : launch_dwconv_ln_swish)(c.big, L.dw, L.ln_dw_g, L.ln_dw_b, c.t1, c.B, c.T, c.stream, SplitOut{})) return rc;
    if (int rc = linear(c, c.t1, kHid, L.pw2, nullptr, c.x, kHid, EPI_NONE, 1.f, c.x, nullptr, kHid)) return rc;
    prof.end(c.stream);
    prof.begin("ffn", 4, c.stream);
    if (int rc = launch_layernorm(c.x, L.ln_ffn2_g, L.ln_ffn2_b, nullptr, c.t1, c.M, kHid, c.stream)) return rc;
    if (int rc = linear(c, c.t1, kHid, L.w2a, L.b2a, c.big, kFfn, EPI_SWISH, 1.f, nullptr, nullptr, kFfn)) return rc;
    if (int rc = linear(c, c.big, kFfn, L.w2b, L.b2b, c.x, kHid, EPI_NONE, 0.5f, c.x, nullptr, kHid)) return rc;
    if (int rc = launch_layernorm(c.x, L.ln_fin_g, L.ln_fin_b, nullptr, c.x, c.M, kHid, c.stream)) return rc;
    prof.end(c.stream);
    return 0;
}

int quantise(const Call& c, int16_t* tokens) {
    const at_w2vbert* h = c.h;
    const SplitCtx sc{scheme_of(h->arith), nullptr};
    c.h->prof.begin("vq", 3, c.stream);
    if (h->arith != ARITH_F32 && h->vq_split && h->cb_s[sc.scheme].p) {
        if (int rc = launch_layernorm_split(c.x, nullptr, nullptr, nullptr, c.t1, c.M, kHid, sc.out(c.t1s, c.Mpad, XB_F16_ACT_SCALE, nullptr), c.stream)) return rc;
        if (int rc = score_split_gemm(sc, c.t1s, h->cb_s[sc.scheme], kCodes, kHid, c.M, c.Mpad, c.big, c.stream)) return rc;
    } else {
        if (int rc = launch_layernorm(c.x, nullptr, nullptr, nullptr, c.t1, c.M, kHid, c.stream)) return rc;
        if (int rc = linear(c, c.t1, kHid, h->codebook, nullptr, c.big, kCodes, EPI_NONE, 1.f, nullptr, nullptr, kCodes)) return rc;
    }
    if (int rc = launch_vq_argmax(c.t1, c.big, h->e2, tokens, c.M, kHid, kCodes, c.stream, c.status, 0, h->vq_refine ? h->codebook : nullptr)) return rc;
    c.h->prof.end(c.stream);
    return 0;
}

}

extern "C" {

int at_w2vbert_encode(at_w2vbert_t* h, const float* wav, const float* mask, int B, int N, int pad_to_multiple_of, int n_layers,
                      int16_t* tokens, int* T_out, float* features_out, float* attn_mask_out, float* hidden_out, void* workspace,
                      size_t workspace_bytes, at_stream_t stream_) {
    return at_w2vbert_encode_checked(h, wav, mask, B, N, pad_to_multiple_of, n_layers, tokens, T_out, features_out, attn_mask_out, hidden_out,
                                     workspace, workspace_bytes, stream_, nullptr);
}

int at_w2vbert_encode_checked(at_w2vbert_t* h, const float* wav, const float* mask, int B, int N, int pad_to_multiple_of, int n_layers,
                              int16_t* tokens, int* T_out, float* features_out, float* attn_mask_out, float* hidden_out, void* workspace,
                              size_t workspace_bytes, at_stream_t stream_, int32_t* status_dev) {
    AT_REQUIRE(h && h->finalized, "model not finalized");
    DeviceGuard guard(h->device);
    AT_REQUIRE(guard.ok, "cannot select the handle's device");
    AT_REQUIRE(wav && workspace, "null pointer");
    AT_REQUIRE(B >= 1 && N >= kFrame + kHop, "need B >= 1 and at least two frames (N >= 560 samples)");
    AT_REQUIRE(n_layers >= 0 && n_layers <= (int)h->layers.size(), "n_layers exceeds the loaded layers");
    AT_REQUIRE(tokens == nullptr || h->codebook != nullptr, "tokens requested but no VQ codebook loaded");
    hipStream_t stream = (hipStream_t)stream_;
    const Plan p = make_plan(B, N, pad_to_multiple_of);
    AT_REQUIRE(workspace_bytes >= p.total_floats * sizeof(float), "workspace too small");
    AT_REQUIRE(p.Tp >= 1, "clip too short");
    if (T_out) *T_out = p.Tp;
    if (status_dev) AT_CHECK_HIP(hipMemsetAsync(status_dev, 0, sizeof(int32_t), stream));
    AT_REQUIRE(n_layers <= kRangeLayers, "more conformer layers than range-table rows");
    if (int rc = h->range.reset(stream)) return rc;

    float* ws = (float*)workspace;
    Call c{};
    c.h = h; c.stream = stream; c.B = B; c.N = N; c.F = p.F; c.T = p.Tp; c.n_layers = n_layers;
    c.M = (long long)B * p.Tp; c.BF = (long long)B * p.F; c.Mpad = (long long)p.Mpad;
    c.status = reinterpret_cast<int*>(status_dev);
    c.frames = reinterpret_cast<double*>(ws + p.off_frames);
    c.fmask = ws + p.off_fmask; c.spec = ws + p.off_spec; c.logmel = ws + p.off_logmel; c.stats = ws + p.off_stats;
    c.feats = features_out ? features_out : ws + p.off_feats;
    c.amask = attn_mask_out ? attn_mask_out : ws + p.off_amask;
    c.x = ws + p.off_x; c.t1 = ws + p.off_t1; c.big = ws + p.off_big;
    c.t1s = reinterpret_cast<piece_t*>(ws + p.off_t1s);
    c.bigs = reinterpret_cast<piece_t*>(ws + p.off_bigs);
    c.kvs = reinterpret_cast<piece_t*>(ws + p.off_kvs);

    if (int rc = front_end(c, wav, mask)) return rc;
    if (int rc = feature_projection(c)) return rc;
    for (int li = 0; li < n_layers; ++li)
        if (int rc = h->arith != ARITH_F32 ? conformer_layer_split(c, li) : conformer_layer_f32(c, li)) return rc;
    if (status_dev)
        if (int rc = launch_range_combine(h->range.dev, n_layers * (int)W_NSITES, c.status, stream)) return rc;
    if (hidden_out) AT_CHECK_HIP(hipMemcpyAsync(hidden_out, c.x, (size_t)c.M * kHid * sizeof(float), hipMemcpyDeviceToDevice, stream));
    if (tokens)
        if (int rc = quantise(c, tokens)) return rc;
    return 0;
}

int at_w2vbert_range_report(at_w2vbert_t* h, float* max_scaled, int cap) { return sem_range_report(h, "at_w2vbert_range_report", max_scaled, cap); }
int at_w2vbert_layer_status(at_w2vbert_t* h, int32_t* flags, int cap) { return sem_layer_status(h, "at_w2vbert_layer_status", flags, cap); }
int at_w2vbert_site_scales(const at_w2vbert_t* h, float* scales, int cap) {
    AT_REQUIRE(h && h->finalized && scales, "at_w2vbert_site_scales: bad arguments");
    const int n = (int)h->layers.size() * (int)W_NSITES;
    AT_REQUIRE(cap >= n, "at_w2vbert_site_scales: buffer too small");
    for (size_t l = 0; l < h->layers.size(); ++l)
        for (int k = 0; k < (int)W_NSITES; ++k) scales[l * W_NSITES + k] = h->layers[l].site_scale[k];
    return n;
}
int at_w2vbert_range_sites(char* names, size_t cap) { return range_sites(kWSiteNames, (int)W_NSITES, names, cap); }

}
```

audiotoken_amd/csrc/w2vbert_kernels.h:

```cpp
#pragma once
#include "at_common.h"
#include "gemm_bf16x3.h"

namespace at {

int launch_frame_prep(const float* wav, const float* smask, const float* window, double* frames, float* fmask, int B, int N,
                      int F, hipStream_t stream, int* status = nullptr);
int launch_dft_f64(const double* frames, const double* dft, float* spec, long long M, int N, hipStream_t stream);
int launch_fbank_normalize(const float* logmel, const float* fmask, float* stats, float* feats, float* amask, int B, int F, int Tp,
                           hipStream_t stream);
int launch_layernorm(const float* x, const float* gamma, const float* beta, const float* row_mask, float* y, long long rows, int D,
                     hipStream_t stream);
struct AttnArgs {
    const float* qkv = nullptr;
    const float* amask = nullptr;
    const float* dist_emb = nullptr;
    float* ctx = nullptr;
    int B = 0, T = 0, heads = 16;
    int arith = -1;
    int* status = nullptr;
    piece_t* ctx_pieces = nullptr;
    long long rows_pad = 0;
    const piece_t* kv_pieces = nullptr;
    int w8 = -1;
    SplitW dist;
};
int launch_relpos_attention(const AttnArgs& a, hipStream_t stream);
int launch_relpos_attention_x3(const AttnArgs& a, int scheme, hipStream_t stream);
bool relpos_attention_w8_eligible(int T, int heads, long long rows_pad, long long B, bool relpos);
int launch_relpos_attention_w8(const AttnArgs& a, hipStream_t stream);
int launch_dist_split(const float* dist_emb, __bf16* out, float scale, hipStream_t stream);
int launch_kv_rowmajor_split(const float* qkv, __bf16* out, long long rows, long long rows_pad, int hid, int* status, hipStream_t stream);
int launch_dwconv_ln_swish(const float* g, const float* w, const float* gamma, const float* beta, float* out, int B, int T, hipStream_t stream,
                           const SplitOut& split = {});
int launch_dwconv_stream(const float* g, const float* w, const float* gamma, const float* beta, float* out, int B, int T, hipStream_t stream,
                         const SplitOut& split = {});
int launch_layernorm_split(const float* x, const float* gamma, const float* beta, const float* row_mask, float* y, long long rows, int D, const SplitOut& split,
                           hipStream_t stream);
int launch_layernorm2_split(const float* x, const float* gamma, const float* beta, float* y, const float* gamma2, const float* beta2, long long rows, int D,
                            const SplitOut& split, hipStream_t stream);
int launch_vq_argmax(const float* x, const float* dots, const float* e2, int16_t* out, long long rows, int D, int C,
                     hipStream_t stream, int* status = nullptr, int ld = 0, const float* codebook = nullptr);

}
```

include/audiotoken_hip.h:

```cpp
#ifndef AUDIOTOKEN_HIP_H
#define AUDIOTOKEN_HIP_H

#include <stddef.h>
#include <stdint.h>

#ifdef __cplusplus
extern "C" {
#endif

typedef void* at_stream_t;

int at_version(void);
const char* at_last_error(void);

typedef struct at_encodec at_encodec_t;

at_encodec_t* at_encodec_create(int device_id);

int at_encodec_set_tensor(at_encodec_t* h, const char* name, const float* host_data, const int64_t* shape, int ndim);

int at_encodec_finalize(at_encodec_t* h, int with_decoder);
void at_encodec_destroy(at_encodec_t* h);
int at_encodec_num_codebooks(const at_encodec_t* h);

size_t at_encodec_workspace_bytes(const at_encodec_t* h, int B, int N);

int at_encodec_encode(at_encodec_t* h, const float* wav, const float* mask, int B, int N, int n_q, int16_t* codes,
                      int* T_out, float* emb_out, void* workspace, size_t workspace_bytes, at_stream_t stream);

int at_encodec_encode_checked(at_encodec_t* h, const float* wav, const float* mask, int B, int N, int n_q, int16_t* codes,
                              int* T_out, float* emb_out, void* workspace, size_t workspace_bytes, at_stream_t stream,
                              uint32_t* status_dev);

size_t at_encodec_stream_state_bytes(const at_encodec_t* h, int B);
int at_encodec_stream_reset(at_encodec_t* h, void* state_dev, int B, at_stream_t stream);
size_t at_encodec_stream_workspace_bytes(const at_encodec_t* h, int B, int n_new);
int at_encodec_encode_stream_checked(at_encodec_t* h, const void* state_in, void* state_out, const float* wav_new, int B, int n_new, int final,
                                     int n_q, int16_t* codes, int* T_out, float* emb_out, void* workspace, size_t workspace_bytes,
                                     at_stream_t stream, uint32_t* status_dev);

int at_encodec_set_option(at_encodec_t* h, const char* name, int value);
int at_encodec_get_option(const at_encodec_t* h, const char* name);

int at_encodec_profile(at_encodec_t* h, int enable);
int at_encodec_profile_read(at_encodec_t* h, char* names, size_t names_cap, float* total_ms, int* launches, int max_groups);

size_t at_encodec_decode_workspace_bytes(const at_encodec_t* h, int B, int T);

int at_encodec_decode(at_encodec_t* h, const int64_t* codes, int B, int K, int T, float* wav, void* workspace,
                      size_t workspace_bytes, at_stream_t stream);
int at_encodec_decode_checked(at_encodec_t* h, const int64_t* codes, int B, int K, int T, float* wav, void* workspace,
                              size_t workspace_bytes, at_stream_t stream, uint32_t* status_dev);

size_t at_encodec_decode_stream_state_bytes(const at_encodec_t* h, int B);
int at_encodec_decode_stream_reset(at_encodec_t* h, void* state_dev, int B, at_stream_t stream);
size_t at_encodec_decode_stream_workspace_bytes(const at_encodec_t* h, int B, int t_new);
int at_encodec_decode_stream_checked(at_encodec_t* h, const void* state_in, void* state_out, const int64_t* codes_new, int B, int K, int t_new,
                                     float* wav_out, void* workspace, size_t workspace_bytes, at_stream_t stream, uint32_t* status_dev);

int at_encodec_stream_gather(at_encodec_t* h, const void* pool, int S, const int32_t* slots_dev, const int32_t* slots_host, int B, void* state_out,
                             at_stream_t stream);
int at_encodec_stream_scatter(at_encodec_t* h, const void* state_in, int B, const int32_t* slots_dev, const int32_t* slots_host, void* pool, int S,
                              at_stream_t stream);
int at_encodec_decode_stream_gather(at_encodec_t* h, const void* pool, int S, const int32_t* slots_dev, const int32_t* slots_host, int B, void* state_out,
                                    at_stream_t stream);
int at_encodec_decode_stream_scatter(at_encodec_t* h, const void* state_in, int B, const int32_t* slots_dev, const int32_t* slots_host, void* pool, int S,
                                     at_stream_t stream);

typedef struct at_w2vbert at_w2vbert_t;

at_w2vbert_t* at_w2vbert_create(int device_id);

int at_w2vbert_set_tensor(at_w2vbert_t* h, const char* name, const float* host_data, const int64_t* shape, int ndim);
int at_w2vbert_finalize(at_w2vbert_t* h);
int64_t at_w2vbert_packed_bytes(at_w2vbert_t* h);
int64_t at_w2vbert_packed_meta(at_w2vbert_t* h, void* host_dst, int64_t cap);
int at_w2vbert_export_packed(at_w2vbert_t* h, void* device_dst, int64_t bytes, void* stream);
int at_w2vbert_import_packed(at_w2vbert_t* h, const void* host_meta, int64_t meta_bytes, const void* device_src, int64_t bytes, void* stream);
void at_w2vbert_destroy(at_w2vbert_t* h);
int at_w2vbert_num_layers(const at_w2vbert_t* h);

int at_w2vbert_num_tokens(int N, int pad_to_multiple_of);
size_t at_w2vbert_workspace_bytes(const at_w2vbert_t* h, int B, int N, int pad_to_multiple_of);

int at_w2vbert_encode(at_w2vbert_t* h, const float* wav, const float* mask, int B, int N, int pad_to_multiple_of, int n_layers,
                      int16_t* tokens, int* T_out, float* features_out, float* attn_mask_out, float* hidden_out, void* workspace,
                      size_t workspace_bytes, at_stream_t stream);
int at_w2vbert_encode_checked(at_w2vbert_t* h, const float* wav, const float* mask, int B, int N, int pad_to_multiple_of, int n_layers,
                              int16_t* tokens, int* T_out, float* features_out, float* attn_mask_out, float* hidden_out, void* workspace,
                              size_t workspace_bytes, at_stream_t stream, int32_t* status_dev);
int at_w2vbert_set_option(at_w2vbert_t* h, const char* name, int value);
int at_w2vbert_get_option(const at_w2vbert_t* h, const char* name);
int at_w2vbert_profile(at_w2vbert_t* h, int enable);
int at_w2vbert_profile_read(at_w2vbert_t* h, char* names, size_t names_cap, float* total_ms, int* launches, int max_groups);

typedef struct at_hubert at_hubert_t;
at_hubert_t* at_hubert_create(int device_id);
int at_hubert_set_tensor(at_hubert_t* h, const char* name, const float* host_data, const int64_t* shape, int ndim);
int at_hubert_finalize(at_hubert_t* h);
int64_t at_hubert_packed_bytes(at_hubert_t* h);
int64_t at_hubert_packed_meta(at_hubert_t* h, void* host_dst, int64_t cap);
int at_hubert_export_packed(at_hubert_t* h, void* device_dst, int64_t bytes, void* stream);
int at_hubert_import_packed(at_hubert_t* h, const void* host_meta, int64_t meta_bytes, const void* device_src, int64_t bytes, void* stream);
void at_hubert_destroy(at_hubert_t* h);
int at_hubert_num_layers(const at_hubert_t* h);
int at_hubert_num_tokens(int N);
size_t at_hubert_workspace_bytes(const at_hubert_t* h, int B, int N);
int at_hubert_encode(at_hubert_t* h, const float* wav, const float* mask, int B, int N, int n_layers, int16_t* tokens, int* T_out,
                     float* hidden_out, void* workspace, size_t workspace_bytes, at_stream_t stream);
int at_hubert_encode_checked(at_hubert_t* h, const float* wav, const float* mask, int B, int N, int n_layers, int16_t* tokens, int* T_out,
                             float* hidden_out, void* workspace, size_t workspace_bytes, at_stream_t stream, int32_t* status_dev);
int at_hubert_features(at_hubert_t* h, const float* wav, int B, int N, float* feats_out, void* workspace, size_t workspace_bytes, at_stream_t stream,
                       int32_t* status_dev);
int at_hubert_set_option(at_hubert_t* h, const char* name, int value);
int at_hubert_get_option(const at_hubert_t* h, const char* name);
int at_hubert_profile(at_hubert_t* h, int enable);
int at_hubert_profile_read(at_hubert_t* h, char* names, size_t names_cap, float* total_ms, int* launches, int max_groups);

int at_flac_info(const uint8_t* data, size_t n, int* sample_rate, int* channels, int* bits_per_sample, int64_t* total_samples, uint8_t* md5_16);
int64_t at_flac_decode(const uint8_t* data, size_t n, int32_t* out, int64_t cap_samples_per_channel);

enum { AT_PCM_S16 = 0, AT_PCM_S32 = 1, AT_PCM_F32 = 2, AT_PCM_U8 = 3 };
typedef struct at_segment_desc {
    const void* pcm;
    const float* table;
    int64_t chunk_off;
    int32_t chunk_len, out_start, valid_len, fmt;
    float scale;
    int32_t o, n, width;
    int32_t chunk_out_len;
} at_segment_desc;
int at_segments_from_pcm(const at_segment_desc* descs_dev, int nseg, int seg_len, float pad_value, float* segments, float* masks, at_stream_t stream);
size_t at_segments_zmuv_workspace_bytes(int nseg, int max_chunk_out_len);
int at_segments_from_pcm_zmuv(const at_segment_desc* descs_dev, int nseg, int seg_len, int max_chunk_out_len, float pad_value, float eps, float* segments,
                              float* masks, void* workspace, size_t workspace_bytes, at_stream_t stream);

typedef struct at_resample_row {
    const void* pcm;
    const float* table;
    int64_t src_base, src_len, src_total, out_start;
    int32_t out_len, fmt;
    float scale;
    int32_t o, n, width, final;
    int32_t reserved;
    int64_t dst_off;
} at_resample_row;
int at_resample_rows(const at_resample_row* rows_dev, int nrows, float* out, at_stream_t stream);
int at_resample_rows_check(const at_resample_row* rows_host, int nrows);

typedef struct at_pcm_row_desc {
    int64_t src_off, dst_off, n;
    float scale;
    int32_t reserved;
} at_pcm_row_desc;
int at_pcm_peaks(const float* src, const at_pcm_row_desc* rows_dev, int nrows, int64_t max_n, float* peaks, at_stream_t stream);
int at_pcm_pack(const float* src, const at_pcm_row_desc* rows_dev, int nrows, int64_t max_n, float limit, int16_t* dst, uint32_t* counts, at_stream_t stream);

enum { AT_FLAC_BLOCK = 4096 };
enum { AT_FLAC_CONSTANT = 0, AT_FLAC_VERBATIM = 1, AT_FLAC_FIXED = 2 };
typedef struct at_flac_row_desc {
    int64_t src_off, n;
    int32_t first_block;
    float scale;
} at_flac_row_desc;
typedef struct at_flac_block {
    int64_t first, byte_off;
    int32_t row, n, kind, order, porder, nbytes;
} at_flac_block;
size_t at_flac_encode_workspace_bytes(int nblocks);
int at_flac_encode_rows(const float* src, const at_flac_row_desc* rows_dev, int nrows, int nblocks, float limit, at_flac_block* blocks, uint8_t* bytes,
                        int64_t bytes_cap, uint32_t* counts, void* workspace, size_t workspace_bytes, at_stream_t stream);
int64_t at_flac_encode_pcm16(const int16_t* samples, int64_t n, int row, at_flac_block* blocks, int64_t blocks_cap, uint8_t* bytes, int64_t bytes_cap,
                             int64_t byte_off);
int64_t at_flac_write_frames(const at_flac_block* blocks, int nblocks, const uint8_t* bytes, int64_t bytes_len, int sample_rate, const int64_t* first_sample_of_row,
                             int nrows, uint8_t* out, int64_t cap, int64_t* stats);
int at_flac_streaminfo(int sample_rate, int min_block, int max_block, int min_frame, int max_frame, int64_t total_samples, uint8_t* out42);

int at_clock_stamp(uint64_t* slots_dev, at_stream_t stream);


int at_encodec_range_sites(char* names, size_t cap);
int at_encodec_range_report(at_encodec_t* h, float* max_scaled, int cap);
int at_w2vbert_range_sites(char* names, size_t cap);
int at_w2vbert_range_report(at_w2vbert_t* h, float* max_scaled, int cap);
int at_hubert_range_sites(char* names, size_t cap);
int at_hubert_range_report(at_hubert_t* h, float* max_scaled, int cap);
int at_w2vbert_site_scales(const at_w2vbert_t* h, float* scales, int cap);
int at_hubert_site_scales(const at_hubert_t* h, float* scales, int cap);
int at_w2vbert_layer_status(at_w2vbert_t* h, int32_t* flags, int cap);
int at_hubert_layer_status(at_hubert_t* h, int32_t* flags, int cap);

typedef struct at_gemm_desc {
    const float* X; int64_t x_bstride; int32_t Tin, Cin, ldx;
    int32_t ktaps, stride, pad_left, pad_mode;
    const float* W; const float* bias;
    float* C; int64_t c_bstride; int32_t ldc;
    const float* R; int64_t r_bstride; int32_t ldr;
    int32_t M, N, K, batch;
    int32_t pro;
    int32_t epi;
    float alpha;
    int32_t aux_off;
    const float* row_mask;
} at_gemm_desc;
int at_op_gemm(const at_gemm_desc* d, at_stream_t stream);
int at_op_gemm_dual(const at_gemm_desc* d, const float* X2, int64_t x2_bstride, int ld2, int K1, at_stream_t stream);
int at_op_gemm_route(const at_gemm_desc* d, const float* X2, int64_t x2_bstride, int ld2, int K1, int32_t* out);

int at_required_tensors(const char* model, int n, int with_extras, char* buf, size_t cap);

int at_op_gemm_split(const float* X, const float* W, const float* bias, float* C, int M, int N, int K, int scheme, float w_max_abs,
                     int kernel, void* workspace, size_t workspace_bytes, int32_t* status_dev, at_stream_t stream);
int at_op_conv_split(const float* X, const float* W, const float* bias, float* C, int B, int L, int Cin, int Cout, int ktaps, int stride,
                     float w_max_abs, void* workspace, size_t workspace_bytes, int32_t* status_dev, at_stream_t stream);
int at_op_rvq_encode(const float* x, int64_t rows, int T, const float* codebooks, const float* e2, int n_q,
                     int16_t* codes, at_stream_t stream);
int at_op_rvq_encode_split(const float* x, int64_t rows, int T, const float* codebooks, const float* e2, int n_q, int16_t* codes, int scheme,
                           float cb_max_abs, void* workspace, size_t workspace_bytes, int32_t* status_dev, at_stream_t stream);

int at_op_hub_conv0(const float* wav, const float* w, const float* gamma, const float* beta, float* out, int B, int N, void* workspace,
                    size_t workspace_bytes, at_stream_t stream);
int at_op_hub_frame_mask(const float* smask, float* fmask, int B, int N, int T, at_stream_t stream);

int at_op_layernorm(const float* x, const float* gamma, const float* beta, const float* row_mask, float* y, int64_t rows, int D,
                    at_stream_t stream);

int at_op_relpos_attention(const float* qkv, const float* attn_mask, const float* dist_emb80, float* ctx, int B, int T,
                           at_stream_t stream);

int at_op_attention_f32(const float* qkv, const float* attn_mask, const float* dist_emb80, float* ctx, int B, int T, int heads, at_stream_t stream);

int at_op_relpos_attention_kvp(const float* qkv, const float* attn_mask, const float* dist_emb80, float dist_max_abs, float* ctx, int B, int T, int heads, int w8,
                               void* kv_workspace, size_t kv_workspace_bytes, int32_t* status_dev, at_stream_t stream);

int at_op_dwconv_ln_swish(const float* g, const float* w31x1024, const float* gamma, const float* beta, float* out, int B, int T,
                          at_stream_t stream);
int at_op_dwconv_stream(const float* g, const float* w31x1024, const float* gamma, const float* beta, float* out, int B, int T,
                        at_stream_t stream);

int at_op_vq_argmax(const float* x, const float* dots, const float* e2, int16_t* out, int64_t rows, int D, int C, at_stream_t stream);
int at_op_vq_argmax_refined(const float* x, const float* dots, const float* e2, const float* codebook, int16_t* out, int64_t rows, int D, int C, at_stream_t stream);

typedef struct at_kmeans at_kmeans_t;

size_t at_kmeans_device_bytes(int64_t N, int D, int K);
at_kmeans_t* at_kmeans_create(int device, int64_t N, int D, int K);
void at_kmeans_destroy(at_kmeans_t* h);
int at_kmeans_set_option(at_kmeans_t* h, const char* name, int value);
int at_kmeans_get_option(const at_kmeans_t* h, const char* name);
int at_kmeans_set_data(at_kmeans_t* h, const float* X, float x_max_abs, at_stream_t stream);
int at_kmeans_plusplus(at_kmeans_t* h, const double* uniforms, int trials, float* C_out, int64_t* picked_rows, at_stream_t stream);
int at_kmeans_assign(at_kmeans_t* h, const float* C, float c_max_abs, int16_t* labels, int32_t* status_dev, at_stream_t stream);
int at_kmeans_update(at_kmeans_t* h, const int16_t* labels, const int16_t* prev_labels, const float* C_old, float* C_new, int32_t* counts,
                     double* stats_dev, at_stream_t stream);
int at_kmeans_layernorm(const float* x, float* y, int64_t rows, int D, int split_kernel, void* workspace, size_t workspace_bytes, at_stream_t stream);
int at_kmeans_row_d2(const at_kmeans_t* h, double* out, at_stream_t stream);
int at_kmeans_relocations(const at_kmeans_t* h, int32_t* out, at_stream_t stream);

typedef struct at_gpt at_gpt_t;
at_gpt_t* at_gpt_create(int device_id);
int at_gpt_set_tensor(at_gpt_t* h, const char* name, const float* host_data, const int64_t* shape, int ndim);
int at_gpt_finalize(at_gpt_t* h);
void at_gpt_destroy(at_gpt_t* h);
int at_gpt_num_layers(const at_gpt_t* h);
int at_gpt_vocab(const at_gpt_t* h);
int at_gpt_block_size(const at_gpt_t* h);
size_t at_gpt_state_bytes(const at_gpt_t* h, int B, int max_len);
#define AT_GPT_FINISH_STOP 1
#define AT_GPT_FINISH_MAX_NEW 2
#define AT_GPT_FINISH_BLOCK 3
int at_gpt_generate(at_gpt_t* h, const int32_t* prompts_dev, int prompt_stride, const int32_t* prompt_len, int B, int max_new, float temperature, int top_k,
                    int stop_token, const float* uniforms_dev, const int32_t* allow, int32_t* out_ids_dev, int32_t* out_len_dev, int32_t* finish_dev,
                    float* logits_out_dev, void* state_dev, size_t state_bytes, int max_len, at_stream_t stream, int32_t* status_dev);
int at_gpt_long_num_windows(int N, int S, int H);
size_t at_gpt_long_state_bytes(const at_gpt_t* h, int B, int max_len);
int at_gpt_generate_long(at_gpt_t* h, const int32_t* src_dev, int src_stride, const int32_t* src_len, int B, int S, int H, int r, int semantic_offset,
                         int semantic_vocab, int infer_token, int acoustic_offset, int codebook_size, int stop_token, int max_new, float temperature, int top_k,
                         const float* uniforms_dev, int u_stride, int32_t* out_ids_dev, int out_stride, int32_t* out_len_dev, int32_t* finish_dev,
                         float* logits_out_dev, void* state_dev, size_t state_bytes, int max_len, at_stream_t stream, int32_t* status_dev);
size_t at_gpt_queue_state_bytes(const at_gpt_t* h, int slots, int max_len, int tick_tokens);
int at_gpt_generate_queue(at_gpt_t* h, const int32_t* src_dev, int src_stride, const int32_t* src_len, int n_src, int S, int H, int r, int semantic_offset,
                          int semantic_vocab, int infer_token, int acoustic_offset, int codebook_size, int stop_token, int max_new, float temperature, int top_k,
                          const float* uniforms_dev, int u_stride, int32_t* out_ids_dev, int out_stride, int32_t* out_len_dev, int32_t* finish_dev,
                          float* logits_out_dev, void* state_dev, size_t state_bytes, int max_len, int slots, int tick_tokens, int32_t* trace, int trace_cap,
                          int32_t* n_ticks, int32_t* placement, at_stream_t stream, int32_t* status_dev);
int at_gpt_long_num_windows_prompted(int P, int N, int S, int H);
int at_gpt_generate_long_prompted(at_gpt_t* h, const int32_t* src_dev, int src_stride, const int32_t* src_len, int B, const int32_t* prompt_sem_dev, int p_stride,
                                  const int32_t* prompt_codes_dev, int f_stride, const int32_t* prompt_len, int n_prompts, const int32_t* prompt_of_src, int S, int H,
                                  int r, int semantic_offset, int semantic_vocab, int infer_token, int acoustic_offset, int codebook_size, int stop_token, int max_new,
                                  float temperature, int top_k, const float* uniforms_dev, int u_stride, int32_t* out_ids_dev, int out_stride, int32_t* out_len_dev,
                                  int32_t* finish_dev, float* logits_out_dev, void* state_dev, size_t state_bytes, int max_len, at_stream_t stream, int32_t* status_dev);
int at_gpt_generate_queue_prompted(at_gpt_t* h, const int32_t* src_dev, int src_stride, const int32_t* src_len, int n_src, const int32_t* prompt_sem_dev, int p_stride,
                                   const int32_t* prompt_codes_dev, int f_stride, const int32_t* prompt_len, int n_prompts, const int32_t* prompt_of_src, int S, int H,
                                   int r, int semantic_offset, int semantic_vocab, int infer_token, int acoustic_offset, int codebook_size, int stop_token, int max_new,
                                   float temperature, int top_k, const float* uniforms_dev, int u_stride, int32_t* out_ids_dev, int out_stride, int32_t* out_len_dev,
                                   int32_t* finish_dev, float* logits_out_dev, void* state_dev, size_t state_bytes, int max_len, int slots, int tick_tokens,
                                   int32_t* trace, int trace_cap, int32_t* n_ticks, int32_t* placement, at_stream_t stream, int32_t* status_dev);
int at_op_topk_sample(const float* logits_dev, int B, int V, float temperature, int top_k, const float* uniforms_dev, const int32_t* allow, int32_t* out_dev,
                      at_stream_t stream);
int at_gpt_set_truncation(at_gpt_t* h, float top_p, float min_p);
int at_op_nucleus_sample(const float* logits_dev, int B, int V, float temperature, int top_k, float top_p, float min_p, const float* uniforms_dev,
                         const int32_t* allow, int32_t* out_dev, int32_t* kept_out_dev, float* thresh_out_dev, at_stream_t stream);
size_t at_gpt_score_state_bytes(const at_gpt_t* h, int rows, int max_len, int pass_tokens, int head_rows);
int at_gpt_score(at_gpt_t* h, const int32_t* seq_dev, int seq_stride, const int32_t* seq_len, const int32_t* score_from, int n_rows, float temperature,
                 const int32_t* allow, float* logprob_out_dev, int32_t* rank_out_dev, int out_stride, float* logits_out_dev, void* state_dev, size_t state_bytes,
                 int rows, int max_len, int pass_tokens, int head_rows, at_stream_t stream, int32_t* status_dev);
int at_op_score_rows(const float* logits_dev, int R, int V, const int32_t* targets_dev, float temperature, const int32_t* allow, float* logprob_out_dev,
                     int32_t* rank_out_dev, at_stream_t stream);

typedef struct at_fine at_fine_t;
at_fine_t* at_fine_create(int device_id);
int at_fine_set_tensor(at_fine_t* h, const char* name, const float* host_data, const int64_t* shape, int ndim);
int at_fine_finalize(at_fine_t* h);
void at_fine_destroy(at_fine_t* h);
int at_fine_num_layers(const at_fine_t* h);
int at_fine_hidden(const at_fine_t* h);
int at_fine_block_size(const at_fine_t* h);
int at_fine_has_bias(const at_fine_t* h);
int at_fine_num_windows(const at_fine_t* h, int T);
size_t at_fine_state_bytes(const at_fine_t* h, int B, int max_T);
int at_fine_generate(at_fine_t* h, const int32_t* coarse_dev, int t_stride, const int32_t* lens, int B, float temperature, int greedy,
                     const float* uniforms_dev, int n_max, int32_t* out_dev, float* logits_out_dev, int32_t* window_ids_dev, void* state_dev, size_t state_bytes,
                     int max_T, at_stream_t stream, int32_t* status_dev);
size_t at_fine_queue_state_bytes(const at_fine_t* h, int slots, int max_T);
int at_fine_generate_queue(at_fine_t* h, const int32_t* coarse_dev, const int32_t* lens, int n_rows, float temperature, int greedy, const float* uniforms_dev,
                           int32_t* out_dev, float* logits_out_dev, int32_t* window_ids_dev, void* state_dev, size_t state_bytes, int max_T, int slots,
                           int32_t* trace, int trace_cap, int32_t* n_passes, int32_t* placement, at_stream_t stream, int32_t* status_dev);
int at_fine_num_windows_hist(const at_fine_t* h, int T, int Th);
size_t at_fine_state_bytes_hist(const at_fine_t* h, int B, int max_T, int max_hist);
size_t at_fine_queue_state_bytes_hist(const at_fine_t* h, int slots, int max_T, int max_hist);
int at_fine_generate_hist(at_fine_t* h, const int32_t* coarse_dev, int t_stride, const int32_t* lens, int B, const int32_t* hist_dev, int h_stride,
                          const int32_t* hist_lens, int n_hist, const int32_t* hist_of_row, int max_hist, float temperature, int greedy,
                          const float* uniforms_dev, int n_max, int32_t* out_dev, float* logits_out_dev, int32_t* window_ids_dev, void* state_dev,
                          size_t state_bytes, int max_T, at_stream_t stream, int32_t* status_dev);
int at_fine_generate_queue_hist(at_fine_t* h, const int32_t* coarse_dev, const int32_t* lens, int n_rows, const int32_t* hist_dev, int h_stride,
                                const int32_t* hist_lens, int n_hist, const int32_t* hist_of_row, int max_hist, float temperature, int greedy,
                                const float* uniforms_dev, int32_t* out_dev, float* logits_out_dev, int32_t* window_ids_dev, void* state_dev, size_t state_bytes,
                                int max_T, int slots, int32_t* trace, int trace_cap, int32_t* n_passes, int32_t* placement, at_stream_t stream,
                                int32_t* status_dev);

size_t at_gpt_stream_state_bytes(const at_gpt_t* h, int S, int H, int r);
int at_gpt_stream_push(at_gpt_t* h, void* state_dev, size_t state_bytes, int64_t* pos, const int32_t* ids_dev, int n_new, int final, int S, int H, int r,
                       int semantic_offset, int semantic_vocab, int infer_token, int acoustic_offset, int codebook_size, int stop_token, int max_new,
                       float temperature, int top_k, const float* uniforms_dev, int64_t u_pos0, int64_t u_len, int32_t* out_ids_dev, int out_cap,
                       int32_t* out_len_dev, int32_t* finish_dev, int32_t* windows_run, at_stream_t stream, int32_t* status_dev);
size_t at_fine_stream_state_bytes(const at_fine_t* h);
int at_fine_stream_push(at_fine_t* h, void* state_dev, size_t state_bytes, int64_t* pos, const int32_t* ids_dev, int n_frames, int final, int acoustic_offset,
                        int codebook_size, float temperature, int greedy, const float* uniforms_dev, int u_win0, int u_windows, int64_t* emit_dev,
                        int emit_stride, int32_t* n_emitted, int32_t* windows_run, at_stream_t stream, int32_t* status_dev);
int at_op_fine_handover(const int32_t* ids_dev, int n_frames, int n_pad, int acoustic_offset, int codebook_size, int32_t* work_dev, at_stream_t stream,
                        int32_t* status_dev);

size_t at_gpt_pool_state_bytes(const at_gpt_t* h, int streams, int slots, int max_len, int tick_tokens, int S, int H, int r);
int at_gpt_pool_push(at_gpt_t* h, void* state_dev, size_t state_bytes, int streams, int slots, int max_len, int tick_tokens, int64_t* pos, int n,
                     const int32_t* place, const int32_t* ids_dev, const int32_t* n_new, const int32_t* final, int S, int H, int r, int semantic_offset,
                     int semantic_vocab, int infer_token, int acoustic_offset, int codebook_size, int stop_token, int max_new, float temperature, int top_k,
                     const float* uniforms_dev, int u_stride, const int64_t* u_pos0, int32_t* out_ids_dev, int out_stride, int32_t* out_len_dev,
                     int32_t* finish_dev, float* logits_out_dev, int32_t* windows_run, int32_t* trace, int trace_cap, int32_t* n_ticks, int32_t* n_rounds,
                     int32_t* placement, at_stream_t stream, int32_t* status_dev);
size_t at_fine_pool_state_bytes(const at_fine_t* h, int streams, int fine_slots);
int at_fine_pool_push(at_fine_t* h, void* state_dev, size_t state_bytes, int streams, int fine_slots, int64_t* pos, int n, const int32_t* place,
                      const int32_t* ids_dev, const int64_t* id_off, const int32_t* n_frames, const int32_t* final, int acoustic_offset, int codebook_size,
                      float temperature, int greedy, const float* uniforms_dev, const int32_t* u_cell0, const int32_t* u_win0, const int32_t* u_windows,
                      int64_t* emit_dev, int emit_stride, int32_t* n_emitted, int32_t* windows_run, int32_t* trace, int trace_cap, int32_t* n_passes,
                      at_stream_t stream, int32_t* status_dev);

#ifdef __cplusplus
}
#endif
#endif
```

Baseline: 15730.

## Precompute per-clip attention key-mask tables once; move P split and row-sum into MFMA slots

Adds a front-end kernel that builds each clip's key bias table and tile mask bits once per forward, reusing logmel workspace. Each attention block then copies the table into LDS instead of recomputing it from the mask with per-element atomics. The fallback path now uses ballot so only one lane per wave does the atomic. The softmax row-sum and the hi/lo fp16 split of probabilities are moved out of the softmax and interleaved with S and PV MFMA issue slots. This shrinks the attention prologue and hides VALU work, but it relies on logmel being dead by attention time and raises register pressure.

```diff
diff --git a/audiotoken_amd/_cabi.py b/audiotoken_amd/_cabi.py
--- a/audiotoken_amd/_cabi.py
+++ b/audiotoken_amd/_cabi.py
@@ -168,6 +168,8 @@
     "at_op_relpos_attention": (C.c_int, [C.c_void_p, C.c_void_p, C.c_void_p, C.c_void_p, C.c_int, C.c_int, C.c_void_p]),
     "at_op_relpos_attention_kvp": (C.c_int, [C.c_void_p, C.c_void_p, C.c_void_p, C.c_float, C.c_void_p, C.c_int, C.c_int, C.c_int, C.c_int, C.c_void_p, C.c_size_t,
                                              C.c_void_p, C.c_void_p]),
+    "at_op_attention_key_tables_bytes": (C.c_size_t, [C.c_int, C.c_int]),
+    "at_op_attention_key_tables": (C.c_int, [C.c_void_p, C.c_int, C.c_int, C.c_void_p, C.c_size_t, C.c_void_p]),
     "at_op_dwconv_ln_swish": (C.c_int, [C.c_void_p, C.c_void_p, C.c_void_p, C.c_void_p, C.c_void_p, C.c_int, C.c_int, C.c_void_p]),
     "at_op_dwconv_stream": (C.c_int, [C.c_void_p, C.c_void_p, C.c_void_p, C.c_void_p, C.c_void_p, C.c_int, C.c_int, C.c_void_p]),
     "at_op_vq_argmax": (C.c_int, [C.c_void_p, C.c_void_p, C.c_void_p, C.c_void_p, C.c_int64, C.c_int, C.c_int, C.c_void_p]),
diff --git a/audiotoken_amd/csrc/attention_f16x2_w8.hip b/audiotoken_amd/csrc/attention_f16x2_w8.hip
--- a/audiotoken_amd/csrc/attention_f16x2_w8.hip
+++ b/audiotoken_amd/csrc/attention_f16x2_w8.hip
@@ -58,7 +58,8 @@
 __global__ __launch_bounds__(512 / W8_NQB, W8_NQB == 1 ? 2 : 1) void relpos_attention_w8_kernel(const float* __restrict__ qkv, const float* __restrict__ amask,
                                                                      const _Float16* __restrict__ dist_pieces, float dist_inv_scale, float* __restrict__ ctx, int T, int hid,
                                                                      int* __restrict__ status, _Float16* __restrict__ ctx_pieces, long long rows_pad,
-                                                                     int nheads, int nclips, const _Float16* __restrict__ kv_pieces) {
+                                                                     int nheads, int nclips, const _Float16* __restrict__ kv_pieces,
+                                                                     const float* __restrict__ key_tables) {
     constexpr int NQB = W8_NQB;
     typedef SchemeF16x2 SC;
     typedef _Float16 PT;
@@ -120,13 +121,22 @@
     if (nkt > 1) issue_k(1, 1);
 
     const float FMIN = -3.4028234663852886e38f;
-    if (tid < 2) tmask[tid] = 0;
-    __syncthreads();
-    for (int k = tid; k < nkt * W8_KB; k += NT) {
-        float v = -INFINITY;
-        if (k < T) v = amask[rowbase + k] != 0.f ? 0.f : FMIN;
-        kbt[k] = v;
-        if (v != 0.f) atomicOr(&tmask[k >> 11], 1 << ((k >> 6) & 31));
+    const int ktab_q = nkt * (W8_KB / 4) + 1;
+    constexpr int KT_Q = (64 * (W8_KB / 4) + 1 + NT - 1) / NT;
+    constexpr int KT_K = 64 * W8_KB / NT;
+    f4 ktq[KT_Q];
+    float kam[KT_K];
+    if (key_tables) {
+        const f4* src = reinterpret_cast<const f4*>(key_tables) + (long long)b * ktab_q;
+#pragma unroll
+        for (int j = 0; j < KT_Q; ++j)
+            if (tid + j * NT < ktab_q) ktq[j] = src[tid + j * NT];
+    } else {
+#pragma unroll
+        for (int j = 0; j < KT_K; ++j) {
+            const int k = tid + j * NT;
+            kam[j] = k < T ? amask[rowbase + k] : 1.f;
+        }
     }
     const int lq0 = l0 + wave * QW + l32;
     V8 qpc[NQB][2][4];
@@ -194,6 +204,24 @@
         const int c0 = ((lane & 16) >> 3) + (vp >> 1), sv = (vq >> 1) & 1;
 #pragma unroll
         for (int dt = 0; dt < 2; ++dt) voff[dt] = (4 * hh + vq) * 128 + ((((dt ^ sv) << 2) + c0) << 4) + (vp & 1) * 8;
+    }
+    if (key_tables) {
+#pragma unroll
+        for (int j = 0; j < KT_Q; ++j)
+            if (tid + j * NT < ktab_q) reinterpret_cast<f4*>(kbt)[tid + j * NT] = ktq[j];
+    } else {
+        if (tid < 2) tmask[tid] = 0;
+        __syncthreads();
+#pragma unroll
+        for (int j = 0; j < KT_K; ++j) {
+            const int k = tid + j * NT;
+            if (k < nkt * W8_KB) {
+                const float v = k < T ? (kam[j] != 0.f ? 0.f : FMIN) : -INFINITY;
+                kbt[k] = v;
+                const bool any = __builtin_amdgcn_ballot_w64(v != 0.f) != 0ull;
+                if (any && lane == 0) atomicOr(&tmask[k >> 11], 1 << ((k >> 6) & 31));
+            }
+        }
     }
     asm volatile("s_waitcnt vmcnt(0)" ::: "memory");
     __syncthreads();
@@ -261,6 +289,7 @@
             }
         return mx;
     };
+    float f_mraw[NQB], f_mnew[NQB], f_bias2[NQB], f_rs[NQB], f_cfar[NQB];
     auto softmax_general = [&](f16v (&s)[2], int kt, int qb) {
         const int r0 = kt * W8_KB;
         const int bmin = wl_min + 32 * qb, bmax = bmin + 31;
@@ -274,24 +303,16 @@
         rescale[qb] = resc;
         const float mnew = resc ? fmaxf(mrun[qb], mx) : mrun[qb];
         const float sub = mnew - W8_P_LOG2;
-        float rs = 0.f;
 #pragma unroll
         for (int kh = 0; kh < 2; ++kh)
 #pragma unroll
-            for (int r = 0; r < 16; ++r) {
-                const float p = __builtin_amdgcn_exp2f(s[kh][r] - sub);
-                s[kh][r] = p;
-                rs += p;
-            }
-        rs = w8_pair_sum(rs);
+            for (int r = 0; r < 16; ++r) s[kh][r] = __builtin_amdgcn_exp2f(s[kh][r] - sub);
         alpha[qb] = resc ? __builtin_amdgcn_exp2f(mrun[qb] - mnew) : 1.0f;
-        lrun[qb] = lrun[qb] * alpha[qb] + rs;
-        mrun[qb] = mnew;
-    };
-    float f_mraw[NQB], f_mnew[NQB], f_bias2[NQB], f_rs[NQB], f_cfar[NQB];
+        f_mnew[qb] = mnew;
+    };
     auto stat_slice = [&](f16v (&sa)[2], int qb, int k) {
         if (k < 4) {
-            if (k == 0) { f_mraw[qb] = -INFINITY; f_rs[qb] = 0.f; }
+            if (k == 0) f_mraw[qb] = -INFINITY;
 #pragma unroll
             for (int e = 0; e < 8; ++e) f_mraw[qb] = fmaxf(f_mraw[qb], sa[k >> 1][8 * (k & 1) + e]);
         } else if (k == 4) {
@@ -305,15 +326,32 @@
 #pragma unroll
             for (int e = 0; e < 2; ++e) {
                 const int r = 2 * (k - 5) + e;
-                const float p = __builtin_amdgcn_exp2f(fmaf(S_SCALE2, sa[r >> 4][r & 15], f_bias2[qb]));
-                sa[r >> 4][r & 15] = p;
-                f_rs[qb] += p;
-            }
-        } else if (k == 21) {
+                sa[r >> 4][r & 15] = __builtin_amdgcn_exp2f(fmaf(S_SCALE2, sa[r >> 4][r & 15], f_bias2[qb]));
+            }
+        }
+    };
+    auto rsum_step = [&](const f16v (&s)[2], int qb, int k) {
+        if (k < 8) {
+            if (k == 0) f_rs[qb] = 0.f;
+#pragma unroll
+            for (int e = 0; e < 4; ++e) f_rs[qb] += s[k >> 2][4 * (k & 3) + e];
+        } else {
             const float rs = w8_pair_sum(f_rs[qb]);
             lrun[qb] = lrun[qb] * alpha[qb] + rs;
             mrun[qb] = f_mnew[qb];
         }
+    };
+    typedef unsigned u4_ __attribute__((ext_vector_type(4)));
+    u4_ pp[2][NQB][2];
+    auto split_pair = [&](const f16v (&s)[2], int ks, int qb, int j) {
+        unsigned hi, lo;
+        if constexpr (W8_PP == 2) {
+            w8_split_pair(s[ks >> 1][8 * (ks & 1) + j], s[ks >> 1][8 * (ks & 1) + j + 1], hi, lo);
+            pp[ks & 1][qb][1][j >> 1] = lo;
+        } else {
+            asm("v_cvt_pk_f16_f32 %0, %1, %2" : "=v"(hi) : "v"(s[ks >> 1][8 * (ks & 1) + j]), "v"(s[ks >> 1][8 * (ks & 1) + j + 1]));
+        }
+        pp[ks & 1][qb][0][j >> 1] = hi;
     };
     auto s_tile_softmax = [&](f16v (&sb)[NQB][2], int kbuf, f16v (&sa)[NQB][2]) {
         const unsigned char* Kb = KV + kbuf * W8_TILE_B;
@@ -342,6 +380,11 @@
                     const int sl = (3 * g + t) * NQB + qb;
                     if (sl < 22) stat_slice(sa[0], 0, sl);
                     else if (NQB > 1 && sl < 44) stat_slice(sa[NQB - 1], NQB - 1, sl - 22);
+                    else {
+                        const int fs = sl - 22 * NQB;
+                        split_pair(sa[fs >> 1], 0, fs >> 1, 4 * (fs & 1));
+                        split_pair(sa[fs >> 1], 0, fs >> 1, 4 * (fs & 1) + 2);
+                    }
                     __builtin_amdgcn_sched_barrier(0);
                 }
         }
@@ -349,18 +392,6 @@
     auto pv_split = [&](const f16v (&s)[NQB][2], int vbuf) {
         const unsigned char* Vb = KV + (W8_KBUFS + vbuf) * W8_TILE_B;
         typedef short s4_ __attribute__((__vector_size__(4 * sizeof(short))));
-        typedef unsigned u4_ __attribute__((ext_vector_type(4)));
-        u4_ pp[2][NQB][2];
-        auto split_pair = [&](int ks, int qb, int j) {
-            unsigned hi, lo;
-            if constexpr (W8_PP == 2) {
-                w8_split_pair(s[qb][ks >> 1][8 * (ks & 1) + j], s[qb][ks >> 1][8 * (ks & 1) + j + 1], hi, lo);
-                pp[ks & 1][qb][1][j >> 1] = lo;
-            } else {
-                asm("v_cvt_pk_f16_f32 %0, %1, %2" : "=v"(hi) : "v"(s[qb][ks >> 1][8 * (ks & 1) + j]), "v"(s[qb][ks >> 1][8 * (ks & 1) + j + 1]));
-            }
-            pp[ks & 1][qb][0][j >> 1] = hi;
-        };
         V8 vf[2][2];
         auto load_v = [&](int u) {
 #pragma unroll
@@ -376,10 +407,12 @@
             }
         };
         load_v(0);
-#pragma unroll
-        for (int qb = 0; qb < NQB; ++qb)
-#pragma unroll
-            for (int j = 0; j < 8; j += 2) split_pair(0, qb, j);
+        if constexpr (W8_PP != 2) {
+#pragma unroll
+            for (int qb = 0; qb < NQB; ++qb)
+#pragma unroll
+                for (int k = 0; k < 9; ++k) rsum_step(s[qb], qb, k);
+        }
         asm volatile("s_nop 1");
         __builtin_amdgcn_sched_barrier(0);
 #pragma unroll
@@ -393,7 +426,9 @@
                 for (int qb = 0; qb < NQB; ++qb) {
                     oacc[qb][dt] = SC::mfma(vf[u & 1][SC::prod_a(t)], __builtin_bit_cast(V8, pp[ks & 1][qb][SC::prod_w(t)]), oacc[qb][dt]);
                     const int sl = (dt * (SC::NPROD - T0) + (t - T0)) * NQB + qb;
-                    if (ks + 1 < 4 && sl < 4 * NQB) split_pair(ks + 1, sl >> 2, 2 * (sl & 3));
+                    if (ks + 1 < 4 && sl < 4 * NQB) split_pair(s[sl >> 2], ks + 1, sl >> 2, 2 * (sl & 3));
+                    else if (W8_PP == 2 && ks + 1 < 4) rsum_step(s[(sl - 4 * NQB) >> 1], (sl - 4 * NQB) >> 1, 2 * ks + ((sl - 4 * NQB) & 1));
+                    else if (W8_PP == 2 && sl / NQB < 3) rsum_step(s[sl % NQB], sl % NQB, 6 + sl / NQB);
                     __builtin_amdgcn_sched_barrier(0);
                 }
         }
@@ -426,12 +461,16 @@
                 for (int qb = 0; qb < NQB; ++qb) {
                     f_cfar[qb] = far_left ? c_left[qb] : c_right[qb];
 #pragma unroll
-                    for (int k = 0; k < 22; ++k) stat_slice(sa[qb], qb, k);
+                    for (int k = 0; k < 21; ++k) stat_slice(sa[qb], qb, k);
                 }
             } else {
 #pragma unroll
                 for (int qb = 0; qb < NQB; ++qb) softmax_general(sa[qb], i, qb);
             }
+#pragma unroll
+            for (int qb = 0; qb < NQB; ++qb)
+#pragma unroll
+                for (int j = 0; j < 8; j += 2) split_pair(sa[qb], 0, qb, j);
         }
         __builtin_amdgcn_sched_barrier(0);
         W8_T(4);
@@ -514,11 +553,11 @@
     if (dist_pieces) {
         static LdsAttrFlags lds_attr;
         rc = set_max_dynamic_lds(lds_attr, relpos_attention_w8_kernel<true>, lds_max);
-        if (!rc) hipLaunchKernelGGL((relpos_attention_w8_kernel<true>), grid, dim3(512 / W8_NQB), lds, stream, qkv, amask, dp, dinv, ctx, T, hid, status, cp, rows_pad, heads, B, kp);
+        if (!rc) hipLaunchKernelGGL((relpos_attention_w8_kernel<true>), grid, dim3(512 / W8_NQB), lds, stream, qkv, amask, dp, dinv, ctx, T, hid, status, cp, rows_pad, heads, B, kp, a.key_tables);
     } else {
         static LdsAttrFlags lds_attr;
         rc = set_max_dynamic_lds(lds_attr, relpos_attention_w8_kernel<false>, lds_max);
-        if (!rc) hipLaunchKernelGGL((relpos_attention_w8_kernel<false>), grid, dim3(512 / W8_NQB), lds, stream, qkv, amask, dp, dinv, ctx, T, hid, status, cp, rows_pad, heads, B, kp);
+        if (!rc) hipLaunchKernelGGL((relpos_attention_w8_kernel<false>), grid, dim3(512 / W8_NQB), lds, stream, qkv, amask, dp, dinv, ctx, T, hid, status, cp, rows_pad, heads, B, kp, a.key_tables);
     }
     if (rc) return rc;
     AT_CHECK_HIP(hipGetLastError());
@@ -541,6 +580,30 @@
     return 0;
 }
 
+__global__ __launch_bounds__(256) void key_table_kernel(const float* __restrict__ amask, float* __restrict__ tables, int T) {
+    __shared__ int tm[4];
+    const int nkt = (T + W8_KB - 1) / W8_KB, tid = threadIdx.x;
+    float* out = tables + (long long)blockIdx.x * (nkt * W8_KB + 4);
+    if (tid < 4) tm[tid] = 0;
+    __syncthreads();
+    for (int k = tid; k < nkt * W8_KB; k += 256) {
+        float v = -INFINITY;
+        if (k < T) v = amask[(long long)blockIdx.x * T + k] != 0.f ? 0.f : -3.4028234663852886e38f;
+        out[k] = v;
+        const bool any = __builtin_amdgcn_ballot_w64(v != 0.f) != 0ull;
+        if (any && (tid & 63) == 0) atomicOr(&tm[k >> 11], 1 << ((k >> 6) & 31));
+    }
+    __syncthreads();
+    if (tid < 4) reinterpret_cast<int*>(out + nkt * W8_KB)[tid] = tm[tid];
+}
+size_t relpos_attention_key_table_floats(int T) { return (size_t)((T + W8_KB - 1) / W8_KB) * W8_KB + 4; }
+int launch_relpos_attention_key_tables(const float* amask, float* tables, int B, int T, hipStream_t stream) {
+    AT_REQUIRE(amask && tables && B >= 1 && T >= 1 && T <= 4096, "relpos_attention_key_tables: needs 1 <= T <= 4096 (64 tile bits)");
+    hipLaunchKernelGGL(key_table_kernel, dim3(B), dim3(256), 0, stream, amask, tables, T);
+    AT_CHECK_HIP(hipGetLastError());
+    return 0;
+}
+
 __global__ __launch_bounds__(256) void dist_split_kernel(const float* __restrict__ e, _Float16* __restrict__ out, float scale) {
     const int q = blockIdx.x * 256 + threadIdx.x;
     if (q >= 96 * 16) return;
diff --git a/audiotoken_amd/csrc/semantic_ops.hip b/audiotoken_amd/csrc/semantic_ops.hip
--- a/audiotoken_amd/csrc/semantic_ops.hip
+++ b/audiotoken_amd/csrc/semantic_ops.hip
@@ -46,6 +46,16 @@
     return launch_relpos_attention(a, (hipStream_t)stream);
 }
 
+size_t at_op_attention_key_tables_bytes(int B, int T) {
+    return B >= 1 && T >= 1 && T <= 4096 ? (size_t)B * relpos_attention_key_table_floats(T) * sizeof(float) : 0;
+}
+
+int at_op_attention_key_tables(const float* attn_mask, int B, int T, void* tables, size_t tables_bytes, at_stream_t stream) {
+    AT_REQUIRE(attn_mask && tables && B >= 1 && T >= 1 && T <= 4096, "bad arguments (1 <= T <= 4096)");
+    AT_REQUIRE(tables_bytes >= at_op_attention_key_tables_bytes(B, T), "key tables too small: at_op_attention_key_tables_bytes(B, T)");
+    return launch_relpos_attention_key_tables(attn_mask, static_cast<float*>(tables), B, T, (hipStream_t)stream);
+}
+
 int at_op_dwconv_ln_swish(const float* g, const float* w31x1024, const float* gamma, const float* beta, float* out, int B, int T,
                           at_stream_t stream) {
     AT_REQUIRE(g && w31x1024 && gamma && beta && out && B >= 1 && T >= 1, "bad arguments");
diff --git a/audiotoken_amd/csrc/w2vbert.hip b/audiotoken_amd/csrc/w2vbert.hip
--- a/audiotoken_amd/csrc/w2vbert.hip
+++ b/audiotoken_amd/csrc/w2vbert.hip
@@ -70,8 +70,8 @@
 
 struct Plan {
     int F, Tp;
-    size_t off_frames, off_fmask, off_spec, off_logmel, off_stats, off_feats, off_amask, off_x, off_t1, off_big, off_tok, off_t1s, off_bigs, off_kvs;
-    size_t Mpad;
+    size_t off_frames, off_fmask, off_spec, off_logmel, off_stats, off_feats, off_amask, off_x, off_t1, off_big, off_tok, off_t1s, off_bigs, off_kvs, off_ktab;
+    size_t Mpad, ktab_floats;
     size_t total_floats;
 };
 
@@ -97,6 +97,9 @@
     p.off_t1s = takef(p.Mpad * kHid * 3 / 2);
     p.off_bigs = takef(p.Mpad * kFfn * 3 / 2);
     p.off_kvs = takef(p.Mpad * kHid * 2 * 2 / 2);
+    p.off_ktab = p.off_logmel;
+    p.ktab_floats = p.Tp >= 1 && p.Tp <= 4096 ? (size_t)B * relpos_attention_key_table_floats(p.Tp) : 0;
+    if (p.ktab_floats > BF * kMel) p.ktab_floats = 0;
     p.total_floats = cur;
     return p;
 }
@@ -318,6 +321,7 @@
     double* frames;
     float *fmask, *spec, *logmel, *stats, *feats, *amask, *x, *t1, *big;
     piece_t *t1s, *bigs, *kvs;
+    float* ktab;
     SplitCtx ctx_of(int li) const { return SplitCtx{scheme_of(h->arith_of(li)), h->range.layer_row(li)}; }
 };
 
@@ -356,7 +360,7 @@
 
 int front_end(const Call& c, const float* wav, const float* mask) {
     const at_w2vbert* h = c.h;
-    c.h->prof.begin("frontend", 5, c.stream);
+    c.h->prof.begin("frontend", c.ktab ? 6 : 5, c.stream);
     if (int rc = launch_frame_prep(wav, mask, h->window, c.frames, c.fmask, c.B, c.N, c.F, c.stream, c.status)) return rc;
     if (int rc = launch_dft_f64(c.frames, h->dft64, c.spec, c.BF, kSpecLd, c.stream)) return rc;
     {
@@ -366,6 +370,8 @@
         if (int rc = launch_gemm(a, c.stream)) return rc;
     }
     if (int rc = launch_fbank_normalize(c.logmel, c.fmask, c.stats, c.feats, c.amask, c.B, c.F, c.T, c.stream)) return rc;
+    if (c.ktab)
+        if (int rc = launch_relpos_attention_key_tables(c.amask, c.ktab, c.B, c.T, c.stream)) return rc;
     c.h->prof.end(c.stream);
     return 0;
 }
@@ -394,7 +400,7 @@
     AttnArgs at;
     at.qkv = c.big; at.amask = c.amask; at.dist_emb = L.dist; at.B = c.B; at.T = c.T; at.heads = 16;
     at.arith = kvp ? ARITH_F16X2 : ARITH_BF16X3;
-    at.status = sc.site(WS_ATTENTION); at.ctx_pieces = c.t1s; at.rows_pad = c.Mpad; at.kv_pieces = kvp ? c.kvs : nullptr; at.w8 = c.h->attn_w8; at.dist = L.dist_s;
+    at.status = sc.site(WS_ATTENTION); at.ctx_pieces = c.t1s; at.rows_pad = c.Mpad; at.kv_pieces = kvp ? c.kvs : nullptr; at.w8 = c.h->attn_w8; at.dist = L.dist_s; at.key_tables = c.ktab;
     if (int rc = launch_relpos_attention(at, c.stream)) return rc;
     prof.end(c.stream);
     prof.begin("attn_proj", 1, c.stream);
@@ -540,6 +546,7 @@
     c.t1s = reinterpret_cast<piece_t*>(ws + p.off_t1s);
     c.bigs = reinterpret_cast<piece_t*>(ws + p.off_bigs);
     c.kvs = reinterpret_cast<piece_t*>(ws + p.off_kvs);
+    c.ktab = h->arith != ARITH_F32 && p.ktab_floats ? ws + p.off_ktab : nullptr;
 
     if (int rc = front_end(c, wav, mask)) return rc;
     if (int rc = feature_projection(c)) return rc;
diff --git a/audiotoken_amd/csrc/w2vbert_kernels.h b/audiotoken_amd/csrc/w2vbert_kernels.h
--- a/audiotoken_amd/csrc/w2vbert_kernels.h
+++ b/audiotoken_amd/csrc/w2vbert_kernels.h
@@ -24,11 +24,14 @@
     const piece_t* kv_pieces = nullptr;
     int w8 = -1;
     SplitW dist;
+    const float* key_tables = nullptr;
 };
 int launch_relpos_attention(const AttnArgs& a, hipStream_t stream);
 int launch_relpos_attention_x3(const AttnArgs& a, int scheme, hipStream_t stream);
 bool relpos_attention_w8_eligible(int T, int heads, long long rows_pad, long long B, bool relpos);
 int launch_relpos_attention_w8(const AttnArgs& a, hipStream_t stream);
+size_t relpos_attention_key_table_floats(int T);
+int launch_relpos_attention_key_tables(const float* amask, float* tables, int B, int T, hipStream_t stream);
 int launch_dist_split(const float* dist_emb, __bf16* out, float scale, hipStream_t stream);
 int launch_kv_rowmajor_split(const float* qkv, __bf16* out, long long rows, long long rows_pad, int hid, int* status, hipStream_t stream);
 int launch_dwconv_ln_swish(const float* g, const float* w, const float* gamma, const float* beta, float* out, int B, int T, hipStream_t stream,
diff --git a/include/audiotoken_hip.h b/include/audiotoken_hip.h
--- a/include/audiotoken_hip.h
+++ b/include/audiotoken_hip.h
@@ -232,6 +232,9 @@
 
 int at_op_relpos_attention_kvp(const float* qkv, const float* attn_mask, const float* dist_emb80, float dist_max_abs, float* ctx, int B, int T, int heads, int w8,
                                void* kv_workspace, size_t kv_workspace_bytes, int32_t* status_dev, at_stream_t stream);
+
+size_t at_op_attention_key_tables_bytes(int B, int T);
+int at_op_attention_key_tables(const float* attn_mask, int B, int T, void* tables, size_t tables_bytes, at_stream_t stream);
 
 int at_op_dwconv_ln_swish(const float* g, const float* w31x1024, const float* gamma, const float* beta, float* out, int B, int T,
                           at_stream_t stream);
```

Result: no change. 15790 (median of 6 runs) (+0.4%).
